# 666DZY666/micronet

Hardware: NVIDIA H100
Metric: qat_step_images_per_sec (higher is better)
Workload: dtype f32 (bf16 tensor-core products of exact integer levels / exact bf16 pieces, fp32 accumulate)

## Files before the change

harness/step_profile.py:

```python
import argparse
import json
import os
import re
import subprocess
import sys

sys.path.insert(0, os.path.dirname(os.path.dirname(os.path.abspath(__file__))))

import torch

from harness import train as H

HEADLINE = "nin_gc_wbwtab_w3a2"


def card():
    try:
        return subprocess.run(["nvidia-smi", "--query-gpu=name,power.limit,clocks.max.sm", "--format=csv,noheader"],
                              capture_output=True, text=True, timeout=30).stdout.strip().splitlines()[0]
    except (OSError, subprocess.SubprocessError, IndexError) as e:
        return f"unknown ({type(e).__name__})"


def producer_bytes(rec, terms_dy):
    n, xb, pooled, plane_only, pk_conv = rec["n"], rec["xb"], rec["pool2"], rec["plane_only"], rec["pk_conv"]
    bits = n / 8
    out = {"channel_stats_kernel": n * xb}
    if pooled:
        out["bn_sign_pool_fwd_kernel"] = n * xb + n + n / 4 + bits
        out["bn_sign_pool_bwd_reduce_kernel"] = n * xb + n + n / 4 + bits
        if pk_conv:
            out["bn_sign_pool_bwd_pack_kernel"] = n * xb + n + n / 4 + bits + 2 * n * terms_dy
        else:
            out["bn_sign_pool_bwd_apply_kernel"] = n * xb + n + n / 4 + bits + 4 * n
    else:
        out["bn_sign_packed_fwd_kernel"] = n * xb + 2 * n + bits + (0 if plane_only else 4 * n)
        out["bn_sign_bwd_reduce_kernel"] = n * xb + 4 * n + bits
        if pk_conv:
            out["bn_sign_bwd_pack_kernel"] = n * xb + 4 * n + bits + 2 * n * terms_dy
        else:
            out["bn_sign_bwd_apply_kernel"] = n * xb + 4 * n + bits + 4 * n
    return out


def base_name(kernel):
    head = kernel.split("(")[0]
    head = re.sub(r"<.*$", "", head)
    return head.split("::")[-1].split(" ")[-1]


def main():
    ap = argparse.ArgumentParser()
    ap.add_argument("--out", required=True)
    ap.add_argument("--steps", type=int, default=5)
    ap.add_argument("--warmup", type=int, default=5)
    ap.add_argument("--batch", type=int, default=256)
    args = ap.parse_args()
    if not torch.cuda.is_available():
        raise SystemExit("step_profile: no CUDA device")
    os.makedirs(args.out, exist_ok=True)
    from micronet_b200 import _lib as L
    from micronet_b200.fused import BatchNormBinarize2d
    w = H.WORKLOADS[HEADLINE]
    dev = torch.device("cuda:0")
    model = H.prepare_engine(H.build_float_model(w["model"]), w["scheme"], **w["prepare"], **w.get("engine_extra", {})).to(dev)
    stepper = H.QatStepper(model, lr=0.01, wd=w["wd"], flat=True, graph=False)
    batches = [H.synthetic_batch(args.batch, w["hw"], seed=100 + i, device=dev) for i in range(2)]
    for i in range(args.warmup):
        stepper.step(*batches[i % 2])
    torch.cuda.synchronize()

    calls = []

    def hook(mod, inp):
        x = inp[0]
        calls.append({"n": x.numel(), "xb": 2 if getattr(x, "_mnb_codes", None) is not None else 4,
                      "pool2": bool(mod.pool2), "plane_only": bool(mod.plane_only) and not mod.pool2,
                      "pk_conv": getattr(x, "_mnb_pk_conv", None) is not None})

    handles = [m.register_forward_pre_hook(hook) for m in model.modules() if isinstance(m, BatchNormBinarize2d)]
    acts = [torch.profiler.ProfilerActivity.CPU, torch.profiler.ProfilerActivity.CUDA]
    with torch.profiler.profile(activities=acts) as prof:
        for i in range(args.steps):
            stepper.step(*batches[i % 2])
        torch.cuda.synchronize()
    for h in handles:
        h.remove()

    terms_dy = min(L.PK_TERMS, L.PK_TERMS_BWD)
    want = {}
    for rec in calls:
        for k, b in producer_bytes(rec, terms_dy).items():
            want[k] = want.get(k, 0.0) + b
    kern = {}
    for e in prof.events():
        if e.device_type != torch.autograd.DeviceType.CUDA:
            continue
        d = kern.setdefault(e.name, {"launches": 0, "us": 0.0})
        d["launches"] += 1
        d["us"] += e.device_time
    rows, total_us = [], sum(d["us"] for d in kern.values()) / args.steps
    for name, d in kern.items():
        row = {"kernel": name, "base": base_name(name), "launches_per_step": d["launches"] / args.steps,
               "us_per_step": d["us"] / args.steps}
        rows.append(row)
    by_base = {}
    for r in rows:
        by_base.setdefault(r["base"], []).append(r)
    for base, rs in by_base.items():
        if base not in want:
            continue
        launches = sum(r["launches_per_step"] for r in rs)
        bytes_step = want[base] / args.steps
        us = sum(r["us_per_step"] for r in rs)
        for r in rs:
            r["bytes_per_launch"] = bytes_step / launches
        rs[0]["group_bytes_per_step"] = bytes_step
        rs[0]["group_GBps"] = bytes_step / (us * 1e-6) / 1e9
    rows.sort(key=lambda r: -r["us_per_step"])
    res = {"card": card(), "workload": HEADLINE, "batch": args.batch, "steps": args.steps,
           "device_us_per_step": total_us, "kernels": rows}
    with open(os.path.join(args.out, "step_profile.json"), "w") as f:
        json.dump(res, f, indent=1)
    lines = [f"card: {res['card']}", f"{HEADLINE}, batch {args.batch}, eager step, {args.steps} profiled steps; "
             f"device time per step {total_us / 1e3:.3f} ms (sum of kernel times)", "",
             f"{'us/step':>9} {'share':>6} {'launch':>6} {'MB/launch':>9} {'GB/s':>7}  kernel"]
    for r in rows:
        mb = f"{r['bytes_per_launch'] / 1e6:9.1f}" if "bytes_per_launch" in r else " " * 9
        gbs = f"{r['group_GBps']:7.0f}" if "group_GBps" in r else " " * 7
        lines.append(f"{r['us_per_step']:9.1f} {r['us_per_step'] / total_us:6.1%} {r['launches_per_step']:6.1f} {mb} {gbs}  "
                     f"{r['kernel'][:110]}")
    txt = "\n".join(lines)
    with open(os.path.join(args.out, "step_profile.txt"), "w") as f:
        f.write(txt + "\n")
    print(txt)


if __name__ == "__main__":
    main()
```

include/micronet_b200.h:

```cpp
#ifndef MICRONET_B200_H
#define MICRONET_B200_H

#include <stdint.h>

#ifdef __cplusplus
extern "C" {
#endif

typedef void* mnb_stream_t;

#define MNB_E_ARG (-1)
#define MNB_E_UNSUPPORTED (-2)

int mnb_version(void);
const char* mnb_last_error(void);
int64_t mnb_launch_count(void);

typedef struct {
  int32_t batch, in_c, in_h, in_w;
  int32_t out_c, ker_h, ker_w;
  int32_t stride_h, stride_w, pad_h, pad_w, dil_h, dil_w, groups;
} mnb_conv_shape;

#define MNB_ACT_DOREFA 1
// ... 103 lines not shown
                    mnb_stream_t stream);
int mnb_bn_sign_bwd(const float* g, const uint32_t* pass_bits, const float* x, int32_t batch, int32_t channels, int32_t hw,
                    const float* mean, const float* invstd, const float* gamma, int32_t training,
                    int32_t out_shuffle_groups, float* dx, float* dgamma, float* dbeta, float* dx_channel_sum,
                    void* scratch, mnb_stream_t stream);

int mnb_bn_sign_pool_fwd(const float* x, int32_t batch, int32_t channels, int32_t H, int32_t W, const float* mean,
                         const float* invstd, const float* gamma, const float* beta, int32_t out_shuffle_groups, float* y,
                         uint32_t* pass_bits, uint8_t* argmax, mnb_stream_t stream);
int mnb_bn_sign_pool_bwd(const float* g, const uint32_t* pass_bits, const uint8_t* argmax, const float* x, int32_t batch,
                         int32_t channels, int32_t H, int32_t W, const float* mean, const float* invstd, const float* gamma,
                         int32_t training, int32_t out_shuffle_groups, float* dx, float* dgamma, float* dbeta,
                         float* dx_channel_sum, void* scratch, mnb_stream_t stream);

int mnb_maxpool2d_fwd(const float* x, int32_t batch, int32_t channels, int32_t H, int32_t W, int32_t kernel, int32_t stride,
                      int32_t pad, int32_t out_shuffle_groups, float* y, uint8_t* argmax, mnb_stream_t stream);
int mnb_maxpool2d_bwd(const float* g, const uint8_t* argmax, int32_t batch, int32_t channels, int32_t H, int32_t W,
                      int32_t kernel, int32_t stride, int32_t pad, int32_t out_shuffle_groups, float* dx,
                      mnb_stream_t stream);

int mnb_bn_sign_fwd_packed(const float* x, int32_t batch, int32_t channels, int32_t hw, const float* mean,
                           const float* invstd, const float* gamma, const float* beta, int32_t out_shuffle_groups, float* y,
                           uint32_t* pass_bits, void* x_packed, mnb_stream_t stream);

int mnb_fconv2d_plan(const mnb_conv_shape* s, int32_t wgrad, int32_t* out, int32_t n);
int mnb_fconv2d_fwd_tc(const mnb_conv_shape* s, const float* x, const float* w, const float* bias, float* y,
                       int32_t* err_flag, mnb_stream_t stream);
int mnb_fconv2d_wg_plan(const mnb_conv_shape* s, int32_t* out, int32_t n);
int mnb_fconv2d_fwd_wg(const mnb_conv_shape* s, const float* x, const float* w, const float* bias, float* y,
                       int32_t* err_flag, mnb_stream_t stream);
int64_t mnb_fconv2d_wgrad_tc_scratch_bytes(const mnb_conv_shape* s);
int64_t mnb_fconv2d_wgrad_wg_scratch_bytes(const mnb_conv_shape* s);
int mnb_fconv2d_wgrad_wg(const mnb_conv_shape* s, const float* dy, const float* x, float* dw, void* scratch,
                         int32_t* err_flag, mnb_stream_t stream);
int mnb_fconv2d_wgrad_tc(const mnb_conv_shape* s, const float* dy, const float* x, float* dw, void* scratch,
                         int32_t* err_flag, mnb_stream_t stream);

int64_t mnb_pk_act_bytes(int32_t batch, int32_t channels, int32_t h, int32_t w, int32_t terms);
int mnb_pk_pack_act(const float* x, int32_t batch, int32_t channels, int32_t h, int32_t w, const mnb_act_qparams* qp,
                    int32_t terms, const float* ch_scale, int32_t phase_split, void* out_pk, uint8_t* bits8,
                    mnb_stream_t stream);
int mnb_bn_relu_quant_pack_fwd(const float* x, int32_t batch, int32_t channels, int32_t hw, const float* mean,
                               const float* invstd, const float* gamma, const float* beta, const mnb_act_qparams* qp,
                               int32_t out_shuffle_groups, void* x_packed, uint32_t* pass_bits, mnb_stream_t stream);
int mnb_bn_sign_bwd_pack(const float* g, const uint32_t* pass_bits, const float* x, int32_t batch, int32_t channels, int32_t hw,
                         const float* mean, const float* invstd, const float* gamma, const float* dgamma, const float* dbeta,
                         int32_t out_shuffle_groups, const float* ch_scale, int32_t terms, float* dx, void* dy_packed,
                         mnb_stream_t stream);
int mnb_bn_sign_pool_bwd_pack(const float* g, const uint32_t* pass_bits, const uint8_t* argmax, const float* x, int32_t batch,
                              int32_t channels, int32_t H, int32_t W, const float* mean, const float* invstd,
                              const float* gamma, const float* dgamma, const float* dbeta, int32_t out_shuffle_groups,
                              const float* ch_scale, int32_t terms, void* dy_packed, mnb_stream_t stream);
int mnb_pk_conv_codes(const mnb_conv_shape* s, const void* a_pk, int32_t terms_a, const void* w_img, int32_t terms_w,
                      const float* n_scale, const float* a_scale, float a_scale_const, const float* bias, int32_t level_bound,
                      int16_t* codes, float* dec, int32_t* err_flag, mnb_stream_t stream);
int mnb_codes_decode(const int16_t* codes, const float* dec, int32_t batch, int32_t channels, int32_t hw, float* x,
                     mnb_stream_t stream);
int mnb_bn_batch_stats_codes(const int16_t* codes, const float* dec, int32_t batch, int32_t channels, int32_t hw, double eps,
                             double momentum, float* running_mean, float* running_var, int64_t* num_batches_tracked,
                             float* mean_invstd, void* scratch, mnb_stream_t stream);
int mnb_bn_sign_fwd_packed_codes(const int16_t* codes, const float* dec, int32_t batch, int32_t channels, int32_t hw,
                                 const float* mean, const float* invstd, const float* gamma, const float* beta,
                                 int32_t out_shuffle_groups, float* y, uint32_t* pass_bits, void* x_packed, mnb_stream_t stream);
int mnb_bn_sign_bwd_codes(const float* g, const uint32_t* pass_bits, const int16_t* codes, const float* dec, int32_t batch,
                          int32_t channels, int32_t hw, const float* mean, const float* invstd, const float* gamma,
                          int32_t training, int32_t out_shuffle_groups, float* dx, float* dgamma, float* dbeta,
                          float* dx_channel_sum, void* scratch, mnb_stream_t stream);
int mnb_bn_sign_pool_fwd_codes(const int16_t* codes, const float* dec, int32_t batch, int32_t channels, int32_t H, int32_t W,
                               const float* mean, const float* invstd, const float* gamma, const float* beta,
                               int32_t out_shuffle_groups, float* y, uint32_t* pass_bits, uint8_t* argmax, mnb_stream_t stream);
int mnb_bn_sign_pool_bwd_codes(const float* g, const uint32_t* pass_bits, const uint8_t* argmax, const int16_t* codes,
                               const float* dec, int32_t batch, int32_t channels, int32_t H, int32_t W, const float* mean,
                               const float* invstd, const float* gamma, int32_t training, int32_t out_shuffle_groups, float* dx,
                               float* dgamma, float* dbeta, float* dx_channel_sum, void* scratch, mnb_stream_t stream);
int mnb_bn_sign_bwd_pack_codes(const float* g, const uint32_t* pass_bits, const int16_t* codes, const float* dec, int32_t batch,
                               int32_t channels, int32_t hw, const float* mean, const float* invstd, const float* gamma,
                               const float* dgamma, const float* dbeta, int32_t out_shuffle_groups, const float* ch_scale,
                               int32_t terms, float* dx, void* dy_packed, mnb_stream_t stream);
int mnb_bn_sign_pool_bwd_pack_codes(const float* g, const uint32_t* pass_bits, const uint8_t* argmax, const int16_t* codes,
                                    const float* dec, int32_t batch, int32_t channels, int32_t H, int32_t W, const float* mean,
                                    const float* invstd, const float* gamma, const float* dgamma, const float* dbeta,
                                    int32_t out_shuffle_groups, const float* ch_scale, int32_t terms, void* dy_packed,
                                    mnb_stream_t stream);
int mnb_pk_pack_act_relu(const float* x, int32_t batch, int32_t channels, int32_t h, int32_t w, const mnb_act_qparams* qp,
                         int32_t terms, const float* ch_scale, int32_t phase_split, int32_t relu, void* out_pk,
                         uint8_t* bits8, mnb_stream_t stream);
int64_t mnb_pk_grouped_act_bytes(int32_t batch, int32_t channels, int32_t h, int32_t w, int32_t terms, int32_t groups);
int mnb_pk_pack_act_grouped(const float* x, int32_t batch, int32_t channels, int32_t h, int32_t w, const mnb_act_qparams* qp,
                            int32_t terms, const float* ch_scale, int32_t phase_split, int32_t relu, void* out_pk,
                            uint8_t* bits8, int32_t groups, mnb_stream_t stream);
int mnb_pk_conv_plan(const mnb_conv_shape* s, int32_t mode, int32_t terms_a, int32_t terms_w, int32_t* out16);
int mnb_pk_conv_plan_ex(const mnb_conv_shape* s, int32_t mode, int32_t terms_a, int32_t terms_w, int32_t* out, int32_t n);
int mnb_pk_wgrad_plan(const mnb_conv_shape* s, int32_t terms_dy, int32_t terms_x, int32_t* out, int32_t n);
int64_t mnb_pk_wimage_bytes(const mnb_conv_shape* s, int32_t mode, int32_t terms_a, int32_t terms_w);
int mnb_pk_pack_weight(const mnb_conv_shape* s, int32_t mode, int32_t terms_a, int32_t terms_w, const int16_t* w_int,
                       const float* w_f32, const float* kzero, void* w_img, mnb_stream_t stream);
int mnb_pk_conv(const mnb_conv_shape* s, int32_t mode, const void* a_pk, int32_t terms_a, const void* w_img, int32_t terms_w,
                const float* n_scale, const float* a_scale, float a_scale_const, const float* bias, const uint8_t* bits8,
                float gain, float* out, int32_t* err_flag, mnb_stream_t stream);
typedef struct mnb_pk_post {
  const mnb_act_qparams* q;
  int32_t relu;
  int32_t phase_split;
  void* out_pk;
  const float* bn_mean;
  const float* bn_invstd;
  const float* bn_gamma;
  const float* bn_beta;
  int32_t shuffle_groups;
  int32_t terms_out;
} mnb_pk_post;
int mnb_pk_conv_post(const mnb_conv_shape* s, const void* a_pk, int32_t terms_a, const void* w_img, int32_t terms_w,
                     const float* n_scale, const float* a_scale, float a_scale_const, const float* bias, float* out,
                     const mnb_pk_post* post, int32_t* err_flag, mnb_stream_t stream);
int mnb_quant_add_pack_fwd(const float* a, const float* b, int32_t batch, int32_t channels, int32_t h, int32_t w,
                           const mnb_act_qparams* qp, int32_t relu, float* out, const mnb_pk_post* post, mnb_stream_t stream);
int mnb_pk_conv_post_plan(const mnb_conv_shape* s, int32_t terms_a, int32_t terms_w, int32_t cpu, const mnb_pk_post* post,
                          int32_t* out, int32_t n);
int64_t mnb_pk_i8_act_bytes(int32_t batch, int32_t channels, int32_t h, int32_t w);
int mnb_pk_i8_pack_act(const float* x, int32_t batch, int32_t channels, int32_t h, int32_t w, const mnb_act_qparams* qp,
                       int32_t phase_split, int32_t relu, void* out_pk, mnb_stream_t stream);
int mnb_pk_i8_conv_plan(const mnb_conv_shape* s, int32_t* out, int32_t n);
int64_t mnb_pk_i8_wimage_bytes(const mnb_conv_shape* s);
int mnb_pk_i8_pack_weight(const mnb_conv_shape* s, const int16_t* w_int, void* w_img, mnb_stream_t stream);
int mnb_pk_i8_conv(const mnb_conv_shape* s, const void* a_pk, const void* w_img, const float* n_scale, const float* a_scale,
                   float a_scale_const, const float* bias, float* out, const mnb_pk_post* post, int32_t* err_flag,
                   mnb_stream_t stream);
int mnb_quant_add_pack_i8_fwd(const float* a, const float* b, int32_t batch, int32_t channels, int32_t h, int32_t w,
                              const mnb_act_qparams* qp, int32_t relu, float* out, const mnb_pk_post* post, mnb_stream_t stream);
int mnb_bn_relu_quant_pack_i8_fwd(const float* x, int32_t batch, int32_t channels, int32_t hw, const float* mean,
                                  const float* invstd, const float* gamma, const float* beta, const mnb_act_qparams* qp,
                                  int32_t out_shuffle_groups, void* x_packed, mnb_stream_t stream);
int mnb_pk_plane_maxpool(const void* in_pk, int32_t batch, int32_t channels, int32_t h, int32_t w, int32_t k, int32_t s, int32_t p,
                         int32_t int8, void* out_pk, mnb_stream_t stream);
int mnb_pk_plane_maxpool_requant(const void* in_pk, int32_t batch, int32_t channels, int32_t h, int32_t w, int32_t k, int32_t s,
                                 int32_t p, int32_t int8, const mnb_act_qparams* q_in, const mnb_act_qparams* q_out, void* out_pk,
                                 mnb_stream_t stream);
int mnb_pk_plane_maxpool_terms(const void* in_pk, int32_t batch, int32_t channels, int32_t h, int32_t w, int32_t k, int32_t s,
                               int32_t p, int32_t terms, void* out_pk, mnb_stream_t stream);
int mnb_bn_relu_pack_terms_fwd(const float* x, int32_t batch, int32_t channels, int32_t hw, const float* mean,
                               const float* invstd, const float* gamma, const float* beta, int32_t relu,
                               int32_t out_shuffle_groups, int32_t terms, void* x_packed, mnb_stream_t stream);
int64_t mnb_pk_wgrad_scratch_bytes(const mnb_conv_shape* s, int32_t terms_dy, int32_t terms_x);
int mnb_pk_wgrad(const mnb_conv_shape* s, const void* dy_pk, int32_t terms_dy, const void* x_pk, int32_t terms_x,
                 const float* a_scale, const float* kdiv, float* dw, void* scratch, int32_t* err_flag, mnb_stream_t stream);
int mnb_pk_wgrad_taps_plan(const mnb_conv_shape* s, int32_t terms_dy, int32_t terms_x, int32_t* out, int32_t n);
int mnb_pk_wgrad_taps(const mnb_conv_shape* s, const void* dy_pk, int32_t terms_dy, const void* x_pk, int32_t terms_x,
                      const float* a_scale, const float* kdiv, float* dw, void* scratch, int32_t* err_flag, mnb_stream_t stream);
int mnb_pk_gc3_plan(const mnb_conv_shape* s, int32_t mode, int32_t terms_a, int32_t terms_w, int32_t* out, int32_t n);
int mnb_pk_gc3_conv(const mnb_conv_shape* s, int32_t mode, const void* a_pk, int32_t terms_a, const void* w_img, int32_t terms_w,
                    const float* n_scale, const float* a_scale, float a_scale_const, const float* bias, const uint8_t* bits8,
                    float gain, float* out, int32_t* err_flag, mnb_stream_t stream);
int mnb_pk_gc3_conv_codes(const mnb_conv_shape* s, const void* a_pk, int32_t terms_a, const void* w_img, int32_t terms_w,
                          const float* n_scale, const float* a_scale, float a_scale_const, const float* bias, int32_t level_bound,
                          int16_t* codes, float* dec, int32_t* err_flag, mnb_stream_t stream);

int mnb_xnor_supported(const mnb_conv_shape* s);
int64_t mnb_xnor_act_bytes(int32_t batch, int32_t channels, int32_t h, int32_t w, int32_t groups);
int mnb_xnor_pack_act(const float* x, int32_t batch, int32_t channels, int32_t h, int32_t w, int32_t groups, void* out_bits,
                      mnb_stream_t stream);
int64_t mnb_xnor_wimage_bytes(const mnb_conv_shape* s);
int mnb_xnor_pack_weight(const mnb_conv_shape* s, const int16_t* w_int, void* w_img, mnb_stream_t stream);
int mnb_xnor_conv_fwd(const mnb_conv_shape* s, const void* a_bits, const void* w_img, const float* alpha, const float* bias,
                      float* y, mnb_stream_t stream);
#define MNB_XNOR_BITS 0
#define MNB_XNOR_PM1_BF16 1
// ... 53 lines not shown
```

micronet_b200/_lib.py:

```python
from __future__ import annotations

import ctypes as C
import os

import torch

_HERE = os.path.dirname(os.path.abspath(__file__))
LIB_PATH = os.path.join(_HERE, "lib", "libmicronet_b200.so")

ACT_DOREFA, ACT_IAO, ACT_SIGN = 1, 2, 3


class ConvShape(C.Structure):
    _fields_ = [(n, C.c_int32) for n in (
        "batch", "in_c", "in_h", "in_w", "out_c", "ker_h", "ker_w", "stride_h", "stride_w",
        "pad_h", "pad_w", "dil_h", "dil_w", "groups")]


class ActQParams(C.Structure):
    _fields_ = [("mode", C.c_int32), ("bits", C.c_int32), ("qmin", C.c_int32), ("qmax", C.c_int32),
                ("q_type", C.c_int32), ("scale", C.c_void_p), ("zero_point", C.c_void_p),
                ("obs_min", C.c_void_p), ("obs_max", C.c_void_p)]


# ... 14 lines not shown
class ConvOperands(C.Structure):
    _fields_ = [("a_codes", C.c_void_p), ("a_f32", C.c_void_p), ("a_offset", C.c_int32),
                ("a_offset_zp", C.c_void_p), ("a_scale", C.c_void_p), ("w_int", C.c_void_p),
                ("w_scale", C.c_void_p), ("w_f32", C.c_void_p), ("bias", C.c_void_p)]


_P, _I, _L, _D = C.c_void_p, C.c_int32, C.c_int64, C.c_double
_SHAPE, _ACTQ, _OPS = C.POINTER(ConvShape), C.POINTER(ActQParams), C.POINTER(ConvOperands)

PROTOTYPES = {
    "mnb_version": (C.c_int, []),
    "mnb_last_error": (C.c_char_p, []),
    "mnb_launch_count": (_L, []),
    "mnb_act_quant_fwd": (C.c_int, [_P, _L, _ACTQ, _P, _P, _P, _P]),
    "mnb_act_quant_bwd": (C.c_int, [_P, _P, _L, _ACTQ, _P, _P]),
    "mnb_bn_fold_fwd": (C.c_int, [_P, _I, _I, _P, _P, _P, _P, _P, _D, _P, _P, _P]),
    "mnb_bn_fold_bwd": (C.c_int, [_P, _P, _P, _I, _I, _P, _P, _P, _P, _D, _P, _P, _P]),
    "mnb_bn_fold_running": (C.c_int, [_P, _P, _P, _P, _I, _D, _I, _P]),
    "mnb_quant_add_fwd": (C.c_int, [_P, _P, _L, _ACTQ, _P, _P, _P, _I, _P]),
    "mnb_quant_add_bwd": (C.c_int, [_P, _P, _P, _L, _ACTQ, _P, _P, _P]),
    "mnb_observe_scratch_bytes": (_L, [_L, _I]),
    "mnb_iao_observe": (C.c_int, [_P, _L, _I, _I, _I, _D, _D, _P, _P, _I, _I, _I, _I, _P, _P, _P, _P]),
    "mnb_iao_update_qparams": (C.c_int, [_P, _P, _I, _I, _I, _I, _P, _P, _P]),
    "mnb_dorefa_weight_fwd": (C.c_int, [_P, _L, _I, _I, _P, _P, _P, _P, _P, _P]),
    "mnb_dorefa_weight_bwd": (C.c_int, [_P, _P, _L, _I, _P, _P, _P]),
    "mnb_wb_weight_fwd": (C.c_int, [_P, _I, _I, _I, _I, _P, _P, _P, _P, _P]),
    "mnb_wb_weight_bwd": (C.c_int, [_P, _P, _P, _I, _I, _I, _I, _P, _P]),
    "mnb_iao_weight_fwd": (C.c_int, [_P, _L, _I, _I, _P, _P, _P, _P, _I, _I, _I, _P, _P, _P, _P, _P]),
    "mnb_iao_weight_bwd": (C.c_int, [_P, _P, _P, _L, _I, _I, _P, _P]),
    "mnb_conv2d_fwd": (C.c_int, [_SHAPE, _OPS, _P, _P]),
    "mnb_conv2d_dgrad": (C.c_int, [_SHAPE, _P, _P, _P, _ACTQ, _P, _P]),
    "mnb_wgrad_scratch_bytes": (_L, [_SHAPE]),
    "mnb_conv2d_wgrad": (C.c_int, [_SHAPE, _P, _OPS, _P, _P, _P]),
    "mnb_channel_stats": (C.c_int, [_P, _I, _I, _I, _I, _P, _P, _P]),
    "mnb_channel_stats_bwd": (C.c_int, [_P, _P, _P, _P, _I, _I, _I, _P, _P]),
    "mnb_fq_conv2d_fwd_tc": (C.c_int, [_SHAPE, _P, _ACTQ, _P, _P, _P, _P, _P, _P, _P, _P, _P]),
    "mnb_conv2d_dgrad_tc": (C.c_int, [_SHAPE, _P, _P, _P, _P, _ACTQ, _P, _P, _P, _P]),
    "mnb_tc_conv_plan": (C.c_int, [_SHAPE, _I, _I, _P, _I]),
    "mnb_wgrad_tc_scratch_bytes": (_L, [_SHAPE]),
    "mnb_wgrad_tc_plan": (C.c_int, [_SHAPE, _I, _P, _I]),
    "mnb_conv2d_wgrad_tc": (C.c_int, [_SHAPE, _P, _P, _ACTQ, _P, _P, _P, _P, _P]),
    "mnb_conv2d_wgrad_cond": (C.c_int, [_SHAPE, _P, _OPS, _P, _P, _P, _P]),
    "mnb_bn_batch_stats": (C.c_int, [_P, _I, _I, _I, _D, _D, _P, _P, _P, _P, _P, _P]),
    "mnb_bn_sign_fwd": (C.c_int, [_P, _I, _I, _I, _P, _P, _P, _P, _I, _P, _P, _P]),
    "mnb_bn_sign_bwd": (C.c_int, [_P, _P, _P, _I, _I, _I, _P, _P, _P, _I, _I, _P, _P, _P, _P, _P, _P]),
    "mnb_bn_sign_pool_fwd": (C.c_int, [_P, _I, _I, _I, _I, _P, _P, _P, _P, _I, _P, _P, _P, _P]),
    "mnb_bn_sign_pool_bwd": (C.c_int, [_P, _P, _P, _P, _I, _I, _I, _I, _P, _P, _P, _I, _I, _P, _P, _P, _P, _P, _P]),
    "mnb_bn_sign_fwd_packed": (C.c_int, [_P, _I, _I, _I, _P, _P, _P, _P, _I, _P, _P, _P, _P]),
    "mnb_fconv2d_plan": (C.c_int, [_SHAPE, _I, _P, _I]),
    "mnb_fconv2d_fwd_tc": (C.c_int, [_SHAPE, _P, _P, _P, _P, _P, _P]),
    "mnb_fconv2d_wg_plan": (C.c_int, [_SHAPE, _P, _I]),
    "mnb_fconv2d_fwd_wg": (C.c_int, [_SHAPE, _P, _P, _P, _P, _P, _P]),
    "mnb_fconv2d_wgrad_tc_scratch_bytes": (_L, [_SHAPE]),
    "mnb_fconv2d_wgrad_tc": (C.c_int, [_SHAPE, _P, _P, _P, _P, _P, _P]),
    "mnb_fconv2d_wgrad_wg_scratch_bytes": (_L, [_SHAPE]),
    "mnb_fconv2d_wgrad_wg": (C.c_int, [_SHAPE, _P, _P, _P, _P, _P, _P]),
    "mnb_maxpool2d_fwd": (C.c_int, [_P, _I, _I, _I, _I, _I, _I, _I, _I, _P, _P, _P]),
    "mnb_maxpool2d_bwd": (C.c_int, [_P, _P, _I, _I, _I, _I, _I, _I, _I, _I, _P, _P]),
    "mnb_adam_step": (C.c_int, [_P, _P, _P, _P, _L, C.c_float, C.c_float, C.c_float, C.c_float, C.c_float, _I, _P]),
    "mnb_pk_act_bytes": (_L, [_I, _I, _I, _I, _I]),
    "mnb_pk_pack_act": (C.c_int, [_P, _I, _I, _I, _I, _ACTQ, _I, _P, _I, _P, _P, _P]),
    "mnb_bn_relu_quant_pack_fwd": (C.c_int, [_P, _I, _I, _I, _P, _P, _P, _P, _ACTQ, _I, _P, _P, _P]),
    "mnb_pk_pack_act_relu": (C.c_int, [_P, _I, _I, _I, _I, _ACTQ, _I, _P, _I, _I, _P, _P, _P]),
    "mnb_pk_grouped_act_bytes": (_L, [_I, _I, _I, _I, _I, _I]),
    "mnb_pk_pack_act_grouped": (C.c_int, [_P, _I, _I, _I, _I, _ACTQ, _I, _P, _I, _I, _P, _P, _I, _P]),
    "mnb_pk_conv_plan": (C.c_int, [_SHAPE, _I, _I, _I, _P]),
    "mnb_pk_conv_plan_ex": (C.c_int, [_SHAPE, _I, _I, _I, _P, _I]),
    "mnb_pk_wgrad_plan": (C.c_int, [_SHAPE, _I, _I, _P, _I]),
    "mnb_pk_wimage_bytes": (_L, [_SHAPE, _I, _I, _I]),
    "mnb_pk_pack_weight": (C.c_int, [_SHAPE, _I, _I, _I, _P, _P, _P, _P, _P]),
    "mnb_pk_conv": (C.c_int, [_SHAPE, _I, _P, _I, _P, _I, _P, _P, C.c_float, _P, _P, C.c_float, _P, _P, _P]),
    "mnb_bn_sign_bwd_pack": (C.c_int, [_P, _P, _P, _I, _I, _I, _P, _P, _P, _P, _P, _I, _P, _I, _P, _P, _P]),
    "mnb_bn_sign_pool_bwd_pack": (C.c_int, [_P, _P, _P, _P, _I, _I, _I, _I, _P, _P, _P, _P, _P, _I, _P, _I, _P, _P]),
    "mnb_pk_conv_post": (C.c_int, [_SHAPE, _P, _I, _P, _I, _P, _P, C.c_float, _P, _P, C.POINTER(PkPost), _P, _P]),
    "mnb_pk_conv_post_plan": (C.c_int, [_SHAPE, _I, _I, _I, C.POINTER(PkPost), _P, _I]),
    "mnb_pk_conv_codes": (C.c_int, [_SHAPE, _P, _I, _P, _I, _P, _P, C.c_float, _P, _I, _P, _P, _P, _P]),
    "mnb_codes_decode": (C.c_int, [_P, _P, _I, _I, _I, _P, _P]),
    "mnb_bn_batch_stats_codes": (C.c_int, [_P, _P, _I, _I, _I, _D, _D, _P, _P, _P, _P, _P, _P]),
    "mnb_bn_sign_fwd_packed_codes": (C.c_int, [_P, _P, _I, _I, _I, _P, _P, _P, _P, _I, _P, _P, _P, _P]),
    "mnb_bn_sign_bwd_codes": (C.c_int, [_P, _P, _P, _P, _I, _I, _I, _P, _P, _P, _I, _I, _P, _P, _P, _P, _P, _P]),
    "mnb_bn_sign_pool_fwd_codes": (C.c_int, [_P, _P, _I, _I, _I, _I, _P, _P, _P, _P, _I, _P, _P, _P, _P]),
    "mnb_bn_sign_pool_bwd_codes": (C.c_int, [_P, _P, _P, _P, _P, _I, _I, _I, _I, _P, _P, _P, _I, _I, _P, _P, _P, _P, _P, _P]),
    "mnb_bn_sign_bwd_pack_codes": (C.c_int, [_P, _P, _P, _P, _I, _I, _I, _P, _P, _P, _P, _P, _I, _P, _I, _P, _P, _P]),
    "mnb_bn_sign_pool_bwd_pack_codes": (C.c_int, [_P, _P, _P, _P, _P, _I, _I, _I, _I, _P, _P, _P, _P, _P, _I, _P, _I, _P,
                                                  _P]),
    "mnb_quant_add_pack_fwd": (C.c_int, [_P, _P, _I, _I, _I, _I, _ACTQ, _I, _P, C.POINTER(PkPost), _P]),
    "mnb_pk_i8_act_bytes": (_L, [_I, _I, _I, _I]),
    "mnb_pk_i8_pack_act": (C.c_int, [_P, _I, _I, _I, _I, _ACTQ, _I, _I, _P, _P]),
    "mnb_pk_i8_conv_plan": (C.c_int, [_SHAPE, _P, _I]),
    "mnb_pk_i8_wimage_bytes": (_L, [_SHAPE]),
    "mnb_pk_i8_pack_weight": (C.c_int, [_SHAPE, _P, _P, _P]),
    "mnb_pk_i8_conv": (C.c_int, [_SHAPE, _P, _P, _P, _P, C.c_float, _P, _P, C.POINTER(PkPost), _P, _P]),
    "mnb_quant_add_pack_i8_fwd": (C.c_int, [_P, _P, _I, _I, _I, _I, _ACTQ, _I, _P, C.POINTER(PkPost), _P]),
    "mnb_bn_relu_quant_pack_i8_fwd": (C.c_int, [_P, _I, _I, _I, _P, _P, _P, _P, _ACTQ, _I, _P, _P]),
    "mnb_pk_plane_maxpool": (C.c_int, [_P, _I, _I, _I, _I, _I, _I, _I, _I, _P, _P]),
    "mnb_pk_plane_maxpool_requant": (C.c_int, [_P, _I, _I, _I, _I, _I, _I, _I, _I, _ACTQ, _ACTQ, _P, _P]),
    "mnb_pk_plane_maxpool_terms": (C.c_int, [_P, _I, _I, _I, _I, _I, _I, _I, _I, _P, _P]),
    "mnb_bn_relu_pack_terms_fwd": (C.c_int, [_P, _I, _I, _I, _P, _P, _P, _P, _I, _I, _I, _P, _P]),
    "mnb_pk_wgrad_scratch_bytes": (_L, [_SHAPE, _I, _I]),
    "mnb_pk_wgrad": (C.c_int, [_SHAPE, _P, _I, _P, _I, _P, _P, _P, _P, _P, _P]),
    "mnb_pk_wgrad_taps_plan": (C.c_int, [_SHAPE, _I, _I, _P, _I]),
    "mnb_pk_wgrad_taps": (C.c_int, [_SHAPE, _P, _I, _P, _I, _P, _P, _P, _P, _P, _P]),
    "mnb_pk_gc3_plan": (C.c_int, [_SHAPE, _I, _I, _I, _P, _I]),
    "mnb_pk_gc3_conv": (C.c_int, [_SHAPE, _I, _P, _I, _P, _I, _P, _P, C.c_float, _P, _P, C.c_float, _P, _P, _P]),
    "mnb_pk_gc3_conv_codes": (C.c_int, [_SHAPE, _P, _I, _P, _I, _P, _P, C.c_float, _P, _I, _P, _P, _P, _P]),
    "mnb_xnor_supported": (C.c_int, [_SHAPE]),
    "mnb_xnor_act_bytes": (_L, [_I, _I, _I, _I, _I]),
    "mnb_xnor_pack_act": (C.c_int, [_P, _I, _I, _I, _I, _I, _P, _P]),
    "mnb_xnor_wimage_bytes": (_L, [_SHAPE]),
    "mnb_xnor_pack_weight": (C.c_int, [_SHAPE, _P, _P, _P]),
    "mnb_xnor_conv_fwd": (C.c_int, [_SHAPE, _P, _P, _P, _P, _P, _P]),
    "mnb_xnor_post_bytes": (_L, [_SHAPE, C.POINTER(XnorPost)]),
    "mnb_xnor_conv_post": (C.c_int, [_SHAPE, _P, _P, _P, _P, C.POINTER(XnorPost), _P, _P]),
    "mnb_xnor_pack_act_post": (C.c_int, [_P, _I, _I, _I, _I, C.POINTER(XnorPost), _P, _P]),
    "mnb_xnor_plan": (C.c_int, [_SHAPE, C.POINTER(XnorPost), _P]),
    "mnb_b1_supported": (C.c_int, [_SHAPE]),
    "mnb_b1_act_bytes": (_L, [_I, _I, _I, _I, _I]),
    "mnb_b1_pack_act": (C.c_int, [_P, _I, _I, _I, _I, _I, _P, _P]),
    "mnb_b1_pack_act_post": (C.c_int, [_P, _I, _I, _I, _I, C.POINTER(XnorPost), _P, _P]),
    "mnb_b1_wimage_bytes": (_L, [_SHAPE]),
    "mnb_b1_pack_weight": (C.c_int, [_SHAPE, _P, _P, _P]),
    "mnb_b1_conv_fwd": (C.c_int, [_SHAPE, _P, _P, _P, _P, _P, _P, _P]),
    "mnb_b1_plan": (C.c_int, [_SHAPE, C.POINTER(XnorPost), _P]),
    "mnb_b1_post_bytes": (_L, [_SHAPE, C.POINTER(XnorPost)]),
    "mnb_b1_conv_post": (C.c_int, [_SHAPE, _P, _P, _P, _P, C.POINTER(XnorPost), _P, _P, _P]),
    "mnb_b1_plane_maxpool": (C.c_int, [_P, _I, _I, _I, _I, _I, _I, _I, _I, _P, _P]),
    "mnb_set_tc_profile_buffer": (None, [_P]),
    "mnb_selftest_mma_rate": (C.c_int, [_I, _I, _I, _I, _I, _P, _P, _P]),
    "mnb_selftest_umma": (C.c_int, [_P, _P, _P, _I, _I, _I, _P, _P]),
    "mnb_selftest_tma3d": (C.c_int, [_P, C.POINTER(C.c_int64), C.POINTER(C.c_int32), C.POINTER(C.c_int32), _P, _P, _P]),
}

_lib = None


def load():
    global _lib
    if _lib is not None:
        return _lib
    if not os.path.exists(LIB_PATH):
        raise RuntimeError(
            f"micronet_b200: {LIB_PATH} is missing - build it with `python -m micronet_b200.build` "
            "(there is no CPU / PyTorch fallback for the fake-quant hot path)")
    lib = C.CDLL(LIB_PATH)
    for name, (res, args) in PROTOTYPES.items():
        fn = getattr(lib, name)
        fn.restype, fn.argtypes = res, args
    _lib = lib
    return lib


def check(rc: int, what: str):
    if rc != 0:
        msg = load().mnb_last_error().decode(errors="replace")
        kind = ValueError if rc < 0 else RuntimeError
        raise kind(f"micronet_b200.{what} failed (code {rc}): {msg}")


def ptr(t):
    return None if t is None else t.data_ptr()


def stream():
    return torch.cuda.current_stream().cuda_stream


def require_cuda(*tensors):
    for t in tensors:
        if t is not None and not t.is_cuda:
            raise RuntimeError(
                "micronet_b200: the fake-quant engine runs on CUDA (sm_90a) tensors only; "
                "got a CPU tensor - there is deliberately no CPU fallback")


def require_f32(*tensors):
    for t in tensors:
        if t is not None and t.dtype != torch.float32:
            raise TypeError(f"micronet_b200: fp32 tensors only (the reference's QAT modules are fp32), got {t.dtype}")


def launch_count() -> int:
    return int(load().mnb_launch_count())


_errflags = {}


def tc_err_flag(device):
    key = (device.type, device.index)
    if key not in _errflags:
        _errflags[key] = torch.zeros(1, dtype=torch.int32, device=device)
    return _errflags[key]


def tc_check(device=None):
    for key, flag in _errflags.items():
        code = int(flag.item())
        if code:
            raise RuntimeError(f"micronet_b200: tensor-core pipeline wait timed out (code {code}) on {key}")


E_UNSUPPORTED = -2
KEEP_DEBUG = False
USE_TC = os.environ.get("MNB_DISABLE_TC", "0") != "1"
PK_MODE = os.environ.get("MNB_PK", "auto")
PK_TERMS = int(os.environ.get("MNB_PK_TERMS", "3"))
PK_TERMS_BWD = int(os.environ.get("MNB_PK_TERMS_BWD", "2"))
PK_WBWTAB = os.environ.get("MNB_PK_WBWTAB", "1") == "1"
PK_WG_TAPS = os.environ.get("MNB_PK_WG_TAPS", "1") != "0"
PK_GC3 = os.environ.get("MNB_PK_GC3", "1") != "0"

XNOR_MODE = os.environ.get("MNB_XNOR", "auto")

PLANE_ONLY = os.environ.get("MNB_PLANE_ONLY", "1") == "1"

_scratch = {}


def scratch(device, rows=1):
    lib = load()
    need = int(lib.mnb_observe_scratch_bytes(0, int(rows)))
    key = (device.type, device.index)
    buf = _scratch.get(key)
    if buf is None or buf.numel() < need:
        buf = torch.zeros(max(need, 1 << 20), dtype=torch.uint8, device=device)
        _scratch[key] = buf
    return buf
```

micronet_b200/csrc/mnb_common.cuh:

```cuda
#pragma once
#include <cuda_runtime.h>
#include <float.h>
#include <stdint.h>

#include "../../include/micronet_b200.h"

int mnb_fail(int code, const char* fmt, ...);
void mnb_count_launches(int n);

#define MNB_REQUIRE(cond, ...)                            \
  do {                                                    \
    if (!(cond)) return mnb_fail(MNB_E_ARG, __VA_ARGS__); \
  } while (0)

#define MNB_LAUNCHED(nlaunch)                                                        \
  do {                                                                               \
    mnb_count_launches(nlaunch);                                                     \
    cudaError_t e__ = cudaGetLastError();                                            \
    if (e__ != cudaSuccess) return mnb_fail((int)e__, "%s:%d launch failed: %s", __FILE__, __LINE__, \
                                            cudaGetErrorString(e__));                \
  } while (0)

static inline int mnb_ceil_div(int64_t a, int64_t b) { return (int)((a + b - 1) / b); }
constexpr int MNB_NUM_SMS = 132;


__device__ __forceinline__ float mnb_round_half_away(float v) {
  float r = floorf(__fadd_rn(fabsf(v), 0.5f));
  return v > 0.f ? r : (v < 0.f ? -r : 0.f);
}
__device__ __forceinline__ float mnb_sign0(float v) { return v > 0.f ? 1.f : (v < 0.f ? -1.f : 0.f); }

__device__ __forceinline__ uint32_t mnb_f2ord(float f) {
  uint32_t u = __float_as_uint(f);
  return (u & 0x80000000u) ? ~u : (u | 0x80000000u);
}
__device__ __forceinline__ float mnb_ord2f(uint32_t u) {
  return __uint_as_float((u & 0x80000000u) ? (u & 0x7fffffffu) : ~u);
}

template <typename T, typename Op>
__device__ __forceinline__ T mnb_warp_reduce(T v, Op op) {
#pragma unroll
  for (int o = 16; o > 0; o >>= 1) v = op(v, __shfl_xor_sync(0xffffffffu, v, o));
  return v;
}
template <typename T, typename Op>
__device__ __forceinline__ T mnb_block_reduce(T v, Op op, T identity, T* smem) {
  const int lane = threadIdx.x & 31, wid = threadIdx.x >> 5;
  v = mnb_warp_reduce(v, op);
  __syncthreads();
  if (lane == 0) smem[wid] = v;
  __syncthreads();
  const int nw = (blockDim.x + 31) >> 5;
  T r = (lane < nw) ? smem[lane] : identity;
  r = mnb_warp_reduce(r, op);
  return r;
}
struct MnbMin { template <typename T> __device__ T operator()(T a, T b) const { return a < b ? a : b; } };
struct MnbMax { template <typename T> __device__ T operator()(T a, T b) const { return a > b ? a : b; } };
struct MnbSum { template <typename T> __device__ T operator()(T a, T b) const { return a + b; } };

__device__ __forceinline__ float bn_bwd_centre(float g, float db, float xhat, float dg) {
  return fmaf(-xhat, dg, __fsub_rn(g, db));
}

struct XDec { float s, b; };
template <typename XT> struct XVec;
template <> struct XVec<float> { typedef float t1; typedef float2 t2; typedef float4 t4; };
template <> struct XVec<int16_t> { typedef short t1; typedef short2 t2; typedef short4 t4; };

template <typename XT>
__device__ __forceinline__ XDec x_dec(const float* dec, int channels, int c) {
  if constexpr (sizeof(XT) == 4) return XDec{1.f, 0.f};
  else return XDec{__ldg(dec + c), __ldg(dec + channels + c)};
}
template <typename XT>
__device__ __forceinline__ float x_val(XT q, XDec d) {
  if constexpr (sizeof(XT) == 4) return q;
  else return fmaf((float)q, d.s, d.b);
}
template <int VEC, typename XT>
__device__ __forceinline__ void x_load(const XT* p, XDec d, float (&v)[VEC]) {
  if constexpr (VEC == 1) {
    v[0] = x_val<XT>(__ldg(reinterpret_cast<const typename XVec<XT>::t1*>(p)), d);
  } else if constexpr (VEC == 2) {
    const typename XVec<XT>::t2 t = __ldg(reinterpret_cast<const typename XVec<XT>::t2*>(p));
    v[0] = x_val<XT>(t.x, d); v[1] = x_val<XT>(t.y, d);
  } else {
    static_assert(VEC == 4, "x_load: 1, 2 or 4 elements");
    const typename XVec<XT>::t4 t = __ldg(reinterpret_cast<const typename XVec<XT>::t4*>(p));
    v[0] = x_val<XT>(t.x, d); v[1] = x_val<XT>(t.y, d); v[2] = x_val<XT>(t.z, d); v[3] = x_val<XT>(t.w, d);
  }
}
template <typename XT>
__device__ __forceinline__ float4 x_load4(const XT* p, XDec d) {
  float v[4];
  x_load<4>(p, d, v);
  return make_float4(v[0], v[1], v[2], v[3]);
}

struct MnbActQ {
  int mode, qmin, qmax;
  float s, zp, lo, hi;
  float rinv;
};

// ... 171 lines not shown
```

micronet_b200/csrc/mnb_fused.cu:

```cuda
#include <algorithm>

#include "mnb_common.cuh"

static inline cudaStream_t S(mnb_stream_t s) { return (cudaStream_t)s; }
constexpr int FUSED_SPLITS = 32;

__device__ __forceinline__ uint32_t shuffled_channel(uint32_t c, uint32_t sg, uint32_t cpg) {
  return sg > 1 ? (c % cpg) * sg + c / cpg : c;
}

__global__ void __launch_bounds__(256) bn_sign_fwd_v4_kernel(const float4* __restrict__ x, uint32_t n4, uint32_t channels,
                                                             uint32_t hw4, uint32_t sg, const float* __restrict__ mean,
                                                             const float* __restrict__ invstd, const float* __restrict__ gamma,
                                                             const float* __restrict__ beta, float4* __restrict__ y,
                                                             uint32_t* __restrict__ bits) {
  const uint32_t lane = threadIdx.x & 31;
  const uint32_t stride = gridDim.x * blockDim.x;
  const uint32_t n4_up = (n4 + 31u) & ~31u;
  const uint32_t cpg = channels / sg;
  for (uint32_t i = blockIdx.x * blockDim.x + threadIdx.x; i < n4_up; i += stride) {
    uint32_t nib = 0;
    if (i < n4) {
      const uint32_t plane = i / hw4, off = i - plane * hw4;
      const uint32_t b = plane / channels, c = plane - b * channels;
      const float mu = __ldg(mean + c), sc = __ldg(gamma + c) * __ldg(invstd + c), be = __ldg(beta + c);
      const float4 v = __ldg(x + i);
      const float b0 = fmaf(v.x - mu, sc, be), b1 = fmaf(v.y - mu, sc, be), b2 = fmaf(v.z - mu, sc, be),
                  b3 = fmaf(v.w - mu, sc, be);
      const uint32_t o = (b * channels + shuffled_channel(c, sg, cpg)) * hw4 + off;
      y[o] = make_float4(b0 < 0.f ? -1.f : 1.f, b1 < 0.f ? -1.f : 1.f, b2 < 0.f ? -1.f : 1.f, b3 < 0.f ? -1.f : 1.f);
      nib = (uint32_t)(fabsf(b0) < 1.f) | ((uint32_t)(fabsf(b1) < 1.f) << 1) | ((uint32_t)(fabsf(b2) < 1.f) << 2) |
            ((uint32_t)(fabsf(b3) < 1.f) << 3);
    }
    uint32_t w = nib << (4 * (lane & 7));
    w |= __shfl_xor_sync(0xffffffffu, w, 1);
    w |= __shfl_xor_sync(0xffffffffu, w, 2);
    w |= __shfl_xor_sync(0xffffffffu, w, 4);
    if ((lane & 7) == 0 && i < n4) bits[i >> 3] = w;
  }
}

__global__ void __launch_bounds__(256) bn_sign_fwd_kernel(const float* __restrict__ x, int64_t n, int channels, int hw,
                                                          int sg, const float* __restrict__ mean,
                                                          const float* __restrict__ invstd, const float* __restrict__ gamma,
                                                          const float* __restrict__ beta, float* __restrict__ y,
                                                          uint32_t* __restrict__ bits) {
  const int lane = threadIdx.x & 31;
  const int64_t warp = ((int64_t)blockIdx.x * blockDim.x + threadIdx.x) >> 5;
  const int64_t nwarps = ((int64_t)gridDim.x * blockDim.x) >> 5;
  const uint32_t cpg = (uint32_t)(channels / sg);
  for (int64_t base = warp * 32; base < n; base += nwarps * 32) {
    const int64_t i = base + lane;
    bool pass = false;
    if (i < n) {
      const int64_t plane = i / hw;
      const int c = (int)(plane % channels);
      const float sc = __ldg(gamma + c) * __ldg(invstd + c);
      const float bn = fmaf(__ldg(x + i) - __ldg(mean + c), sc, __ldg(beta + c));
      pass = fabsf(bn) < 1.f;
      const int64_t o = (plane - c + shuffled_channel((uint32_t)c, (uint32_t)sg, cpg)) * hw + (i - plane * hw);
      y[o] = bn < 0.f ? -1.f : 1.f;
    }
    const uint32_t word = __ballot_sync(0xffffffffu, pass);
    if (lane == 0) bits[base >> 5] = word;
  }
}

template <bool VEC, typename XT>
__global__ void __launch_bounds__(256) bn_sign_bwd_reduce_kernel(const float* __restrict__ g, const uint32_t* __restrict__ bits,
                                                                 const XT* __restrict__ x, const float* __restrict__ dec,
                                                                 int batch, int channels, int hw,
                                                                 int sg, const float* __restrict__ mean,
                                                                 const float* __restrict__ invstd, float* __restrict__ dgamma,
                                                                 float* __restrict__ dbeta, uint32_t* counters,
                                                                 double* partial) {
  __shared__ double red[32];
  __shared__ bool last;
  const int c = blockIdx.x, sp = blockIdx.y, nsp = gridDim.y;
  const int oc = (int)shuffled_channel((uint32_t)c, (uint32_t)sg, (uint32_t)(channels / sg));
  const float mu = __ldg(mean + c), is = __ldg(invstd + c);
  const XDec d = x_dec<XT>(dec, channels, c);
  const int b_lo = (int)((int64_t)batch * sp / nsp), b_hi = (int)((int64_t)batch * (sp + 1) / nsp);
  double s1, s2;
  if (VEC) {
    const uint32_t hw4 = (uint32_t)hw >> 2, total = (uint32_t)(b_hi - b_lo) * hw4;
    const float4* g4 = reinterpret_cast<const float4*>(g);
    float f1[2] = {0.f, 0.f}, f2[2] = {0.f, 0.f};
    for (uint32_t t0 = threadIdx.x; t0 < total; t0 += 2 * blockDim.x) {
#pragma unroll
      for (int u = 0; u < 2; ++u) {
        const uint32_t t = t0 + u * blockDim.x;
        if (t < total) {
          const uint32_t b = t / hw4, i = t - b * hw4;
          const uint32_t fi4 = ((uint32_t)(b_lo + b) * channels + c) * hw4 + i;
          const uint32_t go4 = ((uint32_t)(b_lo + b) * channels + oc) * hw4 + i;
          const uint32_t nib = (__ldg(bits + (fi4 >> 3)) >> (4 * (fi4 & 7))) & 15u;
          const float4 gv = __ldg(g4 + go4), xv = x_load4(x + 4 * fi4, d);
          const float g0 = (nib & 1u) ? gv.x : 0.f, g1 = (nib & 2u) ? gv.y : 0.f, g2 = (nib & 4u) ? gv.z : 0.f,
                      g3 = (nib & 8u) ? gv.w : 0.f;
          f1[u] += (g0 + g1) + (g2 + g3);
          f2[u] += (g0 * ((xv.x - mu) * is) + g1 * ((xv.y - mu) * is)) + (g2 * ((xv.z - mu) * is) + g3 * ((xv.w - mu) * is));
        }
      }
    }
    s1 = (double)f1[0] + (double)f1[1];
    s2 = (double)f2[0] + (double)f2[1];
  } else {
    s1 = 0.0; s2 = 0.0;
    for (int b = b_lo; b < b_hi; ++b) {
      const int64_t off = ((int64_t)b * channels + c) * hw, goff = ((int64_t)b * channels + oc) * hw;
      float f1 = 0.f, f2 = 0.f;
      for (int i = threadIdx.x; i < hw; i += blockDim.x) {
        const int64_t fi = off + i;
        const bool pass = (__ldg(bits + (fi >> 5)) >> (fi & 31)) & 1u;
        const float gv = pass ? __ldg(g + goff + i) : 0.f;
        f1 += gv;
        f2 += gv * ((x_val<XT>(__ldg(x + fi), d) - mu) * is);
      }
      s1 += (double)f1; s2 += (double)f2;
    }
  }
  s1 = mnb_block_reduce(s1, MnbSum(), 0.0, red);
  s2 = mnb_block_reduce(s2, MnbSum(), 0.0, red);
  if (threadIdx.x == 0) {
    partial[((int64_t)c * nsp + sp) * 2 + 0] = s1;
    partial[((int64_t)c * nsp + sp) * 2 + 1] = s2;
    __threadfence();
    last = (atomicAdd(counters + c, 1u) == (uint32_t)nsp - 1);
  }
  __syncthreads();
  if (!last || threadIdx.x != 0) return;
  __threadfence();
  s1 = 0.0; s2 = 0.0;
  for (int j = 0; j < nsp; ++j) { s1 += partial[((int64_t)c * nsp + j) * 2]; s2 += partial[((int64_t)c * nsp + j) * 2 + 1]; }
  dbeta[c] = (float)s1;
  dgamma[c] = (float)s2;
  counters[c] = 0;
}

template <bool VEC, typename XT>
__global__ void __launch_bounds__(256) bn_sign_bwd_apply_kernel(const float* __restrict__ g, const uint32_t* __restrict__ bits,
                                                                const XT* __restrict__ x, const float* __restrict__ dec,
                                                                int batch, int channels, int hw,
                                                                int sg, float inv_count, const float* __restrict__ mean,
                                                                const float* __restrict__ invstd, const float* __restrict__ gamma,
                                                                const float* __restrict__ dgamma, const float* __restrict__ dbeta,
                                                                int training, float* __restrict__ dx, float* __restrict__ dx_sum,
                                                                uint32_t* counters, double* partial) {
  __shared__ double red[32];
  __shared__ bool last;
  const int c = blockIdx.x, sp = blockIdx.y, nsp = gridDim.y;
  const int oc = (int)shuffled_channel((uint32_t)c, (uint32_t)sg, (uint32_t)(channels / sg));
  const float mu = __ldg(mean + c), is = __ldg(invstd + c), k = __ldg(gamma + c) * is;
  const float db = training ? __ldg(dbeta + c) * inv_count : 0.f, dg = training ? __ldg(dgamma + c) * inv_count : 0.f;
  const XDec d = x_dec<XT>(dec, channels, c);
  const int b_lo = (int)((int64_t)batch * sp / nsp), b_hi = (int)((int64_t)batch * (sp + 1) / nsp);
  double s;
  if (VEC) {
    const uint32_t hw4 = (uint32_t)hw >> 2, total = (uint32_t)(b_hi - b_lo) * hw4;
    const float4* g4 = reinterpret_cast<const float4*>(g);
    float4* dx4 = reinterpret_cast<float4*>(dx);
    float f[2] = {0.f, 0.f};
    for (uint32_t t0 = threadIdx.x; t0 < total; t0 += 2 * blockDim.x) {
#pragma unroll
      for (int u = 0; u < 2; ++u) {
        const uint32_t t = t0 + u * blockDim.x;
        if (t < total) {
          const uint32_t b = t / hw4, i = t - b * hw4;
          const uint32_t fi4 = ((uint32_t)(b_lo + b) * channels + c) * hw4 + i;
          const uint32_t go4 = ((uint32_t)(b_lo + b) * channels + oc) * hw4 + i;
          const uint32_t nib = (__ldg(bits + (fi4 >> 3)) >> (4 * (fi4 & 7))) & 15u;
          const float4 gv = __ldg(g4 + go4);
          float v0 = (nib & 1u) ? gv.x : 0.f, v1 = (nib & 2u) ? gv.y : 0.f, v2 = (nib & 4u) ? gv.z : 0.f,
                v3 = (nib & 8u) ? gv.w : 0.f;
          if (training) {
            const float4 xv = x_load4(x + 4 * fi4, d);
            v0 = bn_bwd_centre(v0, db, (xv.x - mu) * is, dg);
            v1 = bn_bwd_centre(v1, db, (xv.y - mu) * is, dg);
            v2 = bn_bwd_centre(v2, db, (xv.z - mu) * is, dg);
            v3 = bn_bwd_centre(v3, db, (xv.w - mu) * is, dg);
          }
          const float4 o = make_float4(k * v0, k * v1, k * v2, k * v3);
          dx4[fi4] = o;
          f[u] += (o.x + o.y) + (o.z + o.w);
        }
      }
    }
    s = (double)f[0] + (double)f[1];
  } else {
    s = 0.0;
    for (int b = b_lo; b < b_hi; ++b) {
      const int64_t off = ((int64_t)b * channels + c) * hw, goff = ((int64_t)b * channels + oc) * hw;
      float f = 0.f;
      for (int i = threadIdx.x; i < hw; i += blockDim.x) {
        const int64_t fi = off + i;
        const bool pass = (__ldg(bits + (fi >> 5)) >> (fi & 31)) & 1u;
        float v = pass ? __ldg(g + goff + i) : 0.f;
        if (training) v = bn_bwd_centre(v, db, (x_val<XT>(__ldg(x + fi), d) - mu) * is, dg);
        v = k * v;
        dx[fi] = v;
        f += v;
      }
      s += (double)f;
    }
  }
  if (!dx_sum) return;
  s = mnb_block_reduce(s, MnbSum(), 0.0, red);
  if (threadIdx.x == 0) {
    partial[((int64_t)c * nsp + sp) * 2] = s;
    __threadfence();
    last = (atomicAdd(counters + c, 1u) == (uint32_t)nsp - 1);
  }
  __syncthreads();
  if (!last || threadIdx.x != 0) return;
  __threadfence();
  s = 0.0;
  for (int j = 0; j < nsp; ++j) s += partial[((int64_t)c * nsp + j) * 2];
  dx_sum[c] = (float)s;
  counters[c] = 0;
}

template <typename XT = float>
static bool planes_vectorizable(int64_t n, int hw, const void* a, const void* b, const void* c, const XT* x = nullptr) {
  return (hw & 3) == 0 && n < (1ll << 31) &&
         (((uintptr_t)a | (uintptr_t)b | (uintptr_t)c) & 15) == 0 && ((uintptr_t)x & (4 * sizeof(XT) - 1)) == 0;
}
static int plane_splits(int batch, int64_t per, int channels) {
  const int64_t want = (2 * 8 * MNB_NUM_SMS + channels - 1) / channels;
  return (int)std::max<int64_t>(1, std::min<int64_t>(std::min<int64_t>(std::min<int64_t>(FUSED_SPLITS, batch), per / 2048), want));
}

extern "C" int mnb_bn_sign_fwd(const float* x, int32_t batch, int32_t channels, int32_t hw, const float* mean,
                               const float* invstd, const float* gamma, const float* beta, int32_t out_shuffle_groups,
                               float* y, uint32_t* pass_bits, mnb_stream_t stream) {
  MNB_REQUIRE(x && mean && invstd && gamma && beta && y && pass_bits, "NULL bn_sign_fwd pointer");
  MNB_REQUIRE(batch > 0 && channels > 0 && hw > 0, "bad bn_sign_fwd shape");
  MNB_REQUIRE(out_shuffle_groups >= 1 && channels % out_shuffle_groups == 0, "shuffle groups %d do not divide %d channels",
              out_shuffle_groups, channels);
  const int64_t n = (int64_t)batch * channels * hw;
  int blocks = (int)std::min<int64_t>(mnb_ceil_div(n, 256 * 4), MNB_NUM_SMS * 8);
  if (planes_vectorizable(n, hw, x, y, nullptr))
    bn_sign_fwd_v4_kernel<<<blocks, 256, 0, S(stream)>>>(reinterpret_cast<const float4*>(x), (uint32_t)(n / 4),
                                                         (uint32_t)channels, (uint32_t)(hw / 4), (uint32_t)out_shuffle_groups,
                                                         mean, invstd, gamma, beta, reinterpret_cast<float4*>(y), pass_bits);
  else
    bn_sign_fwd_kernel<<<blocks, 256, 0, S(stream)>>>(x, n, channels, hw, out_shuffle_groups, mean, invstd, gamma, beta, y,
                                                      pass_bits);
  MNB_LAUNCHED(1);
  return 0;
}

template <typename XT>
static int bn_sign_bwd(const float* g, const uint32_t* pass_bits, const XT* x, const float* dec, int32_t batch, int32_t channels,
                       int32_t hw, const float* mean, const float* invstd, const float* gamma, int32_t training,
                       int32_t out_shuffle_groups, float* dx, float* dgamma, float* dbeta, float* dx_channel_sum, void* scratch,
                       mnb_stream_t stream) {
  MNB_REQUIRE(g && pass_bits && x && mean && invstd && gamma && dx && dgamma && dbeta && scratch, "NULL bn_sign_bwd pointer");
  MNB_REQUIRE(batch > 0 && channels > 0 && channels <= 8192 && hw > 0, "bad bn_sign_bwd shape");
  MNB_REQUIRE(out_shuffle_groups >= 1 && channels % out_shuffle_groups == 0, "shuffle groups %d do not divide %d channels",
              out_shuffle_groups, channels);
  const int64_t n = (int64_t)batch * channels * hw;
  const int64_t per = (int64_t)batch * hw;
  const int splits = plane_splits(batch, per, channels);
  uint32_t* counters = reinterpret_cast<uint32_t*>(reinterpret_cast<char*>(scratch) + 16384);
  double* partial = reinterpret_cast<double*>(reinterpret_cast<char*>(scratch) + 49152);
  const dim3 grid(channels, splits);
  const float inv_count = 1.f / (float)per;
  if (planes_vectorizable(n, hw, g, dx, nullptr, x)) {
    bn_sign_bwd_reduce_kernel<true, XT><<<grid, 256, 0, S(stream)>>>(g, pass_bits, x, dec, batch, channels, hw, out_shuffle_groups,
                                                                     mean, invstd, dgamma, dbeta, counters, partial);
    if (training == 2) { MNB_LAUNCHED(1); return 0; }
    bn_sign_bwd_apply_kernel<true, XT><<<grid, 256, 0, S(stream)>>>(g, pass_bits, x, dec, batch, channels, hw, out_shuffle_groups,
                                                                    inv_count, mean, invstd, gamma, dgamma, dbeta, training, dx,
                                                                    dx_channel_sum, counters, partial);
  } else {
    bn_sign_bwd_reduce_kernel<false, XT><<<grid, 256, 0, S(stream)>>>(g, pass_bits, x, dec, batch, channels, hw, out_shuffle_groups,
                                                                      mean, invstd, dgamma, dbeta, counters, partial);
    if (training == 2) { MNB_LAUNCHED(1); return 0; }
    bn_sign_bwd_apply_kernel<false, XT><<<grid, 256, 0, S(stream)>>>(g, pass_bits, x, dec, batch, channels, hw, out_shuffle_groups,
                                                                     inv_count, mean, invstd, gamma, dgamma, dbeta, training, dx,
                                                                     dx_channel_sum, counters, partial);
  }
  MNB_LAUNCHED(2);
  return 0;
}

extern "C" int mnb_bn_sign_bwd(const float* g, const uint32_t* pass_bits, const float* x, int32_t batch, int32_t channels,
                               int32_t hw, const float* mean, const float* invstd, const float* gamma, int32_t training,
                               int32_t out_shuffle_groups, float* dx, float* dgamma, float* dbeta, float* dx_channel_sum,
                               void* scratch, mnb_stream_t stream) {
  return bn_sign_bwd<float>(g, pass_bits, x, nullptr, batch, channels, hw, mean, invstd, gamma, training, out_shuffle_groups, dx,
                            dgamma, dbeta, dx_channel_sum, scratch, stream);
}

extern "C" int mnb_bn_sign_bwd_codes(const float* g, const uint32_t* pass_bits, const int16_t* codes, const float* dec,
                                     int32_t batch, int32_t channels, int32_t hw, const float* mean, const float* invstd,
                                     const float* gamma, int32_t training, int32_t out_shuffle_groups, float* dx, float* dgamma,
                                     float* dbeta, float* dx_channel_sum, void* scratch, mnb_stream_t stream) {
  MNB_REQUIRE(dec, "NULL decode pair");
  return bn_sign_bwd<int16_t>(g, pass_bits, codes, dec, batch, channels, hw, mean, invstd, gamma, training, out_shuffle_groups, dx,
                              dgamma, dbeta, dx_channel_sum, scratch, stream);
}

struct PoolGeom { uint32_t channels, H, W4, OH, OW2, sg; };

__device__ __forceinline__ uint32_t first_max_of_signs(bool p0, bool p1, bool p2, bool p3) {
  return p0 ? 0u : (p1 ? 1u : (p2 ? 2u : (p3 ? 3u : 0u)));
}

template <typename XT>
__global__ void __launch_bounds__(256) bn_sign_pool_fwd_kernel(const XT* __restrict__ x, const float* __restrict__ dec,
                                                               uint32_t n_pairs, PoolGeom gm,
                                                               const float* __restrict__ mean, const float* __restrict__ invstd,
                                                               const float* __restrict__ gamma, const float* __restrict__ beta,
// ... 422 lines not shown
```

micronet_b200/csrc/mnb_pk.cu:

```cuda
#include <cuda.h>
#include <cuda_bf16.h>

#include <algorithm>
#include <cstdlib>
#include <cstring>

#include "mnb_common.cuh"
#include "mnb_tc.cuh"

namespace pk {

constexpr int MAXST = 8;
constexpr int MAXTAP = 64, MAXTMPL = 16, MAXY = 4, MAXPAIR = 6, MAXPROG = 512;
constexpr int kSmemBudget = 227 * 1024 - 3072;
constexpr int kNtSizes[] = {16, 32, 48, 64, 96, 128};

struct Tmpl { int kph, tap0, ntap, blk_off, blk_bytes; };

struct Plan {
  int mode;
  int B, G, R, S, stride;
  int HA, WA, C8A, nkph;
  int kg, ng, NOUT;
  int OHr, OWr, OH, OW, omul, ny;
  int hlo, hhi, wlo, whi;
  int Wt, BW, TH, THH, TB, npos, col_tiles, row_tiles, img_tiles, n_mtiles;
  int Nt, n_ntiles, MT, n_mgroups, n_items;
  int CC, ksteps, chunks;
  int TA, TBk, npairs, pair_a[MAXPAIR], pair_b[MAXPAIR];
  int ntmpl[MAXY], ntap[MAXY];
  Tmpl tmpl[MAXY][MAXTMPL];
  int tap_aoff[MAXY][MAXTAP];
  short tap_r[MAXY][MAXTAP], tap_s[MAXY][MAXTAP];
  int img_bytes[MAXY], y_off[MAXY];
  int64_t wimg_bytes;
  int a_box_bytes, a_bytes, b_off, stage_bytes, nstage, st_log2, smem_bytes, off_stg;
  int segmented, seg_len;
  int cpu;
};

static inline int ceil_div(int a, int b) { return (a + b - 1) / b; }
static inline int round_up(int a, int b) { return ceil_div(a, b) * b; }

static void make_pairs(int TA, int TBk, Plan& p) {
  const int lim = std::max(TA, TBk) - 1;
  p.npairs = 0;
  for (int sum = lim; sum >= 0; --sum)
    for (int a = 0; a < TA; ++a) {
      const int b = sum - a;
      if (b < 0 || b >= TBk) continue;
      if (p.npairs < MAXPAIR) { p.pair_a[p.npairs] = a; p.pair_b[p.npairs] = b; ++p.npairs; }
    }
}

static int unsupported(const char* why) { return mnb_fail(MNB_E_UNSUPPORTED, "pk conv: %s", why); }

static int make_plan(const mnb_conv_shape* s, int mode, int TA, int TBk, Plan& p, int cpu = 8) {
  MNB_REQUIRE(s != nullptr, "conv shape is NULL");
  memset(&p, 0, sizeof(p));
  const int C = s->in_c, K = s->out_c, G = s->groups, H = s->in_h, W = s->in_w, R = s->ker_h, S = s->ker_w;
  MNB_REQUIRE(s->batch > 0 && C > 0 && K > 0 && H > 0 && W > 0 && G > 0 && C % G == 0 && K % G == 0 && R > 0 && S > 0,
              "bad conv shape");
  MNB_REQUIRE(TA >= 1 && TA <= 3 && TBk >= 1 && TBk <= 3, "term counts must be 1..3");
  MNB_REQUIRE(cpu == 8 || (cpu == 16 && mode == 0 && TA == 1 && TBk == 1), "int8 plans are single-product forward plans");
  if (s->dil_h != 1 || s->dil_w != 1) return unsupported("dilation != 1");
  if (s->stride_h != s->stride_w || (s->stride_h != 1 && s->stride_h != 2)) return unsupported("stride must be 1 or 2");
  const int st = s->stride_h, ph_ = s->pad_h, pw_ = s->pad_w;
  if (ph_ > R - 1 || pw_ > S - 1) return unsupported("padding larger than the filter");
  const int P = (H + 2 * ph_ - R) / st + 1, Q = (W + 2 * pw_ - S) / st + 1;
  if (P < 1 || Q < 1) return unsupported("empty output");
  if (st == 2 && ((H | W) & 1)) return unsupported("stride 2 needs even H and W");
  const int cin_g = C / G, cout_g = K / G;
  p.mode = mode; p.B = s->batch; p.G = G; p.R = R; p.S = S; p.stride = st;
  p.TA = TA; p.TBk = TBk; p.cpu = cpu;
  make_pairs(TA, TBk, p);
  if (mode == 0) {
    p.kg = cin_g; p.ng = cout_g; p.NOUT = K;
    p.nkph = st == 2 ? 4 : 1;
    p.HA = H / st; p.WA = W / st; p.C8A = ceil_div(C, cpu);
    p.OHr = P; p.OWr = Q; p.OH = P; p.OW = Q; p.omul = 1; p.ny = 1;
  } else {
    p.kg = cout_g; p.ng = cin_g; p.NOUT = C;
    p.nkph = 1; p.HA = P; p.WA = Q; p.C8A = ceil_div(K, 8);
    p.OHr = H / st; p.OWr = W / st; p.OH = H; p.OW = W; p.omul = st; p.ny = st == 2 ? 4 : 1;
  }
  if (cpu == 16 && G > 1 && (p.kg % cpu)) return unsupported("grouped int8 conv needs GEMM-K channels per group % 16 == 0");
  if (cpu == 8) p.C8A = G * ceil_div(p.kg, 8);
  if (cpu == 16 && (int64_t)p.kg * R * S * 128 * 127 > (int64_t)INT32_MAX) return unsupported("int8 sums could overflow s32");
  struct Tap { int kph, sh, sw, r, s; };
// ... 502 lines not shown
}

__global__ void __launch_bounds__(256) bn_relu_pack_terms_kernel(const float* __restrict__ x, int batch, int channels, int hw,
                                                                 int sg, const float* __restrict__ mean,
                                                                 const float* __restrict__ invstd,
                                                                 const float* __restrict__ gamma,
                                                                 const float* __restrict__ beta, int relu, int terms,
                                                                 uint4* __restrict__ xp) {
  const int c8n = channels / 8, cpg = channels / sg;
  const int64_t total = (int64_t)batch * c8n * hw;
  for (int64_t idx = (int64_t)blockIdx.x * blockDim.x + threadIdx.x; idx < total; idx += (int64_t)gridDim.x * blockDim.x) {
    const int pos = (int)(idx % hw);
    const int64_t t = idx / hw;
    const int oc8 = (int)(t % c8n), b = (int)(t / c8n);
    float v[8];
#pragma unroll
    for (int j = 0; j < 8; ++j) {
      const int oc = oc8 * 8 + j;
      const int c = sg > 1 ? (oc % sg) * cpg + oc / sg : oc;
      float y = __ldg(x + ((int64_t)b * channels + c) * hw + pos);
      if (mean) y = fmaf(__fsub_rn(y, __ldg(mean + c)), __fmul_rn(__ldg(gamma + c), __ldg(invstd + c)), __ldg(beta + c));
      v[j] = relu ? fmaxf(y, 0.f) : y;
    }
    store_terms8(v, terms, xp + idx, total);
  }
}

template <int CPU>
__global__ void __launch_bounds__(256) quant_add_pack_kernel(const float* __restrict__ a, const float* __restrict__ b, int B, int C,
                                                             int H, int W, int C8, mnb_act_qparams qadd, int relu,
                                                             float* __restrict__ out, mnb_act_qparams qnext, int next_relu,
                                                             int phase_split, uint4* __restrict__ out_pk) {
  const MnbActQ q = mnb_load_actq(qadd), qn = mnb_load_actq(qnext);
  const float zpn = (qnext.mode == MNB_ACT_IAO && qnext.zero_point) ? __ldg(qnext.zero_point) : 0.f;
  const uint32_t HW = (uint32_t)H * (uint32_t)W;
  const uint32_t plane = blockIdx.y * blockDim.y + threadIdx.y;
  if (plane >= (uint32_t)B * (uint32_t)C8) return;
  const uint32_t bi = plane / (uint32_t)C8, c8 = plane - bi * (uint32_t)C8;
  for (uint32_t pos = blockIdx.x * blockDim.x + threadIdx.x; pos < HW; pos += gridDim.x * blockDim.x) {
    const int64_t base = ((int64_t)bi * C + c8 * CPU) * HW + pos;
    float va[CPU], vb[CPU], lev[CPU];
#pragma unroll
    for (int j = 0; j < CPU; ++j) {
      const bool live = (int)c8 * CPU + j < C;
      va[j] = live ? __ldg(a + base + (int64_t)j * HW) : 0.f;
      vb[j] = live ? __ldg(b + base + (int64_t)j * HW) : 0.f;
    }
    float la[CPU], lb[CPU], sum[CPU];
    uint32_t pbits;
    mnb_act_levels<CPU>(q, va, la, pbits);
    mnb_act_levels<CPU>(q, vb, lb, pbits);
#pragma unroll
    for (int j = 0; j < CPU; ++j) {
      const bool live = (int)c8 * CPU + j < C;
      float oa, ob;
      if (q.mode == MNB_ACT_DOREFA) { oa = __fmul_rn(la[j], q.s); ob = __fmul_rn(lb[j], q.s); }
      else { oa = __fmul_rn(__fadd_rn(la[j], q.zp), q.s); ob = __fmul_rn(__fadd_rn(lb[j], q.zp), q.s); }
      float t = __fadd_rn(oa, ob);
      if (relu) t = fmaxf(t, 0.f);
      if (live) out[base + (int64_t)j * HW] = t;
      sum[j] = next_relu ? fmaxf(t, 0.f) : t;
    }
    mnb_act_levels<CPU>(qn, sum, lev, pbits);
#pragma unroll
    for (int j = 0; j < CPU; ++j) lev[j] = ((int)c8 * CPU + j < C) ? lev[j] + zpn : 0.f;
    int64_t dst;
    if (phase_split) {
      const uint32_t h = pos / (uint32_t)W, w = pos - h * (uint32_t)W;
      const uint32_t oct = ((h & 1u) * 2u + (w & 1u)) * (uint32_t)C8 + c8;
      dst = (((int64_t)bi * 4 * C8 + oct) * (H >> 1) + (h >> 1)) * (W >> 1) + (w >> 1);
    } else {
      dst = (int64_t)plane * HW + pos;
    }
    if constexpr (CPU == 16) out_pk[dst] = pack16_s8(lev);
    else out_pk[dst] = make_uint4(pack2(lev[0], lev[1]), pack2(lev[2], lev[3]), pack2(lev[4], lev[5]), pack2(lev[6], lev[7]));
  }
}

template <int VEC> struct PkVec;
template <> struct PkVec<1> { typedef float type; };
template <> struct PkVec<2> { typedef float2 type; };
template <> struct PkVec<4> { typedef float4 type; };

template <int VEC, typename XT>
__global__ void __launch_bounds__(256) bn_sign_bwd_pack_kernel(const float* __restrict__ g, const uint32_t* __restrict__ bits,
                                                               const XT* __restrict__ x, const float* __restrict__ dec,
                                                               int batch, int channels, int hw,
                                                               int sg, float inv_count, const float* __restrict__ mean,
                                                               const float* __restrict__ invstd, const float* __restrict__ gamma,
                                                               const float* __restrict__ dgamma, const float* __restrict__ dbeta,
                                                               const float* __restrict__ ch_scale, int terms,
                                                               float* __restrict__ dx, uint4* __restrict__ out, int64_t plane_vecs) {
  typedef typename PkVec<VEC>::type T;
  const int lane = threadIdx.x & 31;
  const int c8n = channels / 8, cpg = channels / sg, chunks = hw / (32 * VEC);
  const int64_t items = (int64_t)batch * c8n * chunks;
  const int64_t nwarps = ((int64_t)gridDim.x * blockDim.x) >> 5;
  for (int64_t w = ((int64_t)blockIdx.x * blockDim.x + threadIdx.x) >> 5; w < items; w += nwarps) {
    const int ch = (int)(w % chunks);
    const int64_t pl = w / chunks;
    const int c8 = (int)(pl % c8n), b = (int)(pl / c8n);
    const int pos = (ch * 32 + lane) * VEC;
    T gv[8];
    float xf[8][VEC];
    uint32_t bw[8];
#pragma unroll
    for (int j = 0; j < 8; ++j) {
      const int c = c8 * 8 + j;
      const int oc = sg > 1 ? (c % cpg) * sg + c / cpg : c;
      const int64_t fi = ((int64_t)b * channels + c) * hw + pos;
      gv[j] = __ldg(reinterpret_cast<const T*>(g + ((int64_t)b * channels + oc) * hw + pos));
      x_load<VEC>(x + fi, x_dec<XT>(dec, channels, c), xf[j]);
      bw[j] = __ldg(bits + (fi >> 5)) >> (fi & 31);
    }
    float v[VEC][8];
#pragma unroll
    for (int j = 0; j < 8; ++j) {
      const int c = c8 * 8 + j;
      const float mu = __ldg(mean + c), is = __ldg(invstd + c), k = __ldg(gamma + c) * is;
      const float db = __ldg(dbeta + c) * inv_count, dg = __ldg(dgamma + c) * inv_count;
      const float sc = ch_scale ? __ldg(ch_scale + c) : 1.f;
      const float* gf = reinterpret_cast<const float*>(&gv[j]);
      T dv;
      float* df = reinterpret_cast<float*>(&dv);
#pragma unroll
      for (int i = 0; i < VEC; ++i) {
        float t = ((bw[j] >> i) & 1u) ? gf[i] : 0.f;
        t = bn_bwd_centre(t, db, (xf[j][i] - mu) * is, dg);
        t = k * t;
        df[i] = t;
        v[i][j] = ch_scale ? __fmul_rn(t, sc) : t;
      }
      if (dx) *reinterpret_cast<T*>(dx + ((int64_t)b * channels + c) * hw + pos) = dv;
    }
    const int64_t dst = pl * hw + pos;
    for (int tm = 0; tm < terms; ++tm) {
#pragma unroll
      for (int i = 0; i < VEC; ++i) {
        uint32_t pk4[4];
#pragma unroll
        for (int j = 0; j < 4; ++j) {
          pk4[j] = pack2(v[i][2 * j], v[i][2 * j + 1]);
          v[i][2 * j] -= __uint_as_float(pk4[j] << 16);
          v[i][2 * j + 1] -= __uint_as_float(pk4[j] & 0xffff0000u);
        }
        out[(int64_t)tm * plane_vecs + dst + i] = make_uint4(pk4[0], pk4[1], pk4[2], pk4[3]);
      }
    }
  }
}

template <typename XT>
__global__ void __launch_bounds__(256) bn_sign_pool_bwd_pack_kernel(const float2* __restrict__ g, const uchar2* __restrict__ arg,
                                                                    const uint8_t* __restrict__ bits8, const XT* __restrict__ x,
                                                                    const float* __restrict__ dec, int batch, int channels, int H, int W4, int sg, float inv_count,
                                                                    const float* __restrict__ mean, const float* __restrict__ invstd,
                                                                    const float* __restrict__ gamma, const float* __restrict__ dgamma,
                                                                    const float* __restrict__ dbeta, const float* __restrict__ ch_scale,
                                                                    int terms, uint4* __restrict__ out, int64_t plane_vecs) {
  const uint32_t OH = (uint32_t)H / 2u, OW2 = (uint32_t)W4, c8n = (uint32_t)channels / 8u, cpg = (uint32_t)channels / (uint32_t)sg;
  const uint32_t per_plane = OH * OW2;
  const int64_t total = (int64_t)batch * c8n * per_plane;
  for (int64_t it = (int64_t)blockIdx.x * blockDim.x + threadIdx.x; it < total; it += (int64_t)gridDim.x * blockDim.x) {
    const uint32_t rem = (uint32_t)(it % per_plane);
    const int64_t pl = it / per_plane;
    const uint32_t c8 = (uint32_t)(pl % c8n), b = (uint32_t)(pl / c8n);
    const uint32_t oh = rem / OW2, j = rem - oh * OW2;
    float v[8][8];
#pragma unroll
    for (int q = 0; q < 8; ++q) {
      const uint32_t c = c8 * 8u + q;
      const uint32_t oc = sg > 1 ? (c % cpg) * (uint32_t)sg + c / cpg : c;
      const uint32_t plane = b * (uint32_t)channels + c;
      const float2 gv = __ldg(g + ((size_t)(b * (uint32_t)channels + oc) * OH + oh) * OW2 + j);
      const uchar2 a = arg[((size_t)plane * OH + oh) * OW2 + j];
      const uint32_t i0 = (plane * (uint32_t)H + 2u * oh) * (uint32_t)W4 + j, i1 = i0 + (uint32_t)W4;
      const uint32_t n0 = (bits8[i0 >> 1] >> (4u * (i0 & 1u))) & 15u, n1 = (bits8[i1 >> 1] >> (4u * (i1 & 1u))) & 15u;
      const XDec d = x_dec<XT>(dec, channels, (int)c);
      const float4 r0 = x_load4(x + 4 * i0, d), r1 = x_load4(x + 4 * i1, d);
      const float mu = __ldg(mean + c), is = __ldg(invstd + c), k = __ldg(gamma + c) * is;
      const float db = __ldg(dbeta + c) * inv_count, dg = __ldg(dgamma + c) * inv_count;
      const float sc = ch_scale ? __ldg(ch_scale + c) : 1.f;
      const uint32_t e0 = (a.x >> 1) * 4u + (a.x & 1u), e1 = (a.y >> 1) * 4u + 2u + (a.y & 1u);
      const uint32_t nib = n0 | (n1 << 4);
      const float xs[8] = {r0.x, r0.y, r0.z, r0.w, r1.x, r1.y, r1.z, r1.w};
#pragma unroll
      for (int e = 0; e < 8; ++e) {
        float t = 0.f;
        if ((uint32_t)e == e0 && ((nib >> e) & 1u)) t = gv.x;
        if ((uint32_t)e == e1 && ((nib >> e) & 1u)) t = gv.y;
        t = bn_bwd_centre(t, db, (xs[e] - mu) * is, dg);
        t = k * t;
        v[e][q] = ch_scale ? __fmul_rn(t, sc) : t;
      }
    }
    const int64_t dst0 = (pl * H + 2 * oh) * (int64_t)(4 * W4) + 4 * j;
    for (int tm = 0; tm < terms; ++tm) {
#pragma unroll
      for (int e = 0; e < 8; ++e) {
        uint32_t pk4[4];
#pragma unroll
        for (int q = 0; q < 4; ++q) {
          pk4[q] = pack2(v[e][2 * q], v[e][2 * q + 1]);
          v[e][2 * q] -= __uint_as_float(pk4[q] << 16);
          v[e][2 * q + 1] -= __uint_as_float(pk4[q] & 0xffff0000u);
        }
        out[(int64_t)tm * plane_vecs + dst0 + (e >> 2) * (int64_t)(4 * W4) + (e & 3)] = make_uint4(pk4[0], pk4[1], pk4[2], pk4[3]);
      }
    }
  }
}

struct PackWParams {
  Plan pl;
  const int16_t* w_int; const float* w_f32; const float* kzero;
  int cin_g, cout_g;
};

template <int CPU>
__global__ void __launch_bounds__(256) pack_weight_kernel(const __grid_constant__ PackWParams pp, uint4* __restrict__ out) {
  const Plan& p = pp.pl;
  const int64_t total = p.wimg_bytes / 16;
  const int RS = p.R * p.S;
  for (int64_t v = (int64_t)blockIdx.x * blockDim.x + threadIdx.x; v < total; v += (int64_t)gridDim.x * blockDim.x) {
    int64_t byte = v * 16;
    int y = 0;
    for (int yy = 1; yy < p.ny; ++yy) if (byte >= p.y_off[yy]) y = yy;
    byte -= p.y_off[y];
    if (p.img_bytes[y] == 0) continue;
    const int ntg = (int)(byte / p.img_bytes[y]);
// ... 1274 lines not shown
                     p.segmented, p.segmented ? p.seg_len : 0, p.npairs, p.col_tiles, p.n_mgroups,
                     p.ntmpl[0], p.ntmpl[1], p.ntmpl[2], p.ntmpl[3], p.ntap[0], p.ntap[1], p.ntap[2], p.ntap[3], words, last_seg};
  for (int i = 0; i < std::min(n, 31); ++i) out[i] = v[i];
}

extern "C" int64_t mnb_pk_act_bytes(int32_t batch, int32_t channels, int32_t h, int32_t w, int32_t terms) {
  return (int64_t)terms * batch * ((channels + 7) / 8) * h * w * 16;
}

extern "C" int mnb_pk_pack_act(const float* x, int32_t batch, int32_t channels, int32_t h, int32_t w,
                               const mnb_act_qparams* qp, int32_t terms, const float* ch_scale, int32_t phase_split,
                               void* out_pk, uint8_t* bits8, mnb_stream_t stream) {
  return mnb_pk_pack_act_relu(x, batch, channels, h, w, qp, terms, ch_scale, phase_split, 0, out_pk, bits8, stream);
}

extern "C" int mnb_pk_pack_act_relu(const float* x, int32_t batch, int32_t channels, int32_t h, int32_t w,
                                    const mnb_act_qparams* qp, int32_t terms, const float* ch_scale, int32_t phase_split,
                                    int32_t relu, void* out_pk, uint8_t* bits8, mnb_stream_t stream) {
  MNB_REQUIRE(x && out_pk, "NULL pk_pack_act pointer");
  MNB_REQUIRE(batch > 0 && channels > 0 && h > 0 && w > 0 && terms >= 1 && terms <= 3, "bad pk_pack_act arguments");
  MNB_REQUIRE((reinterpret_cast<uintptr_t>(out_pk) & 15) == 0, "packed tensor must be 16-byte aligned");
  if (phase_split) MNB_REQUIRE(((h | w) & 1) == 0, "phase split needs even H and W");
  const int C8 = (channels + 7) / 8;
  const int64_t plane_vecs = (int64_t)batch * C8 * h * w;
  MNB_REQUIRE((int64_t)batch * C8 <= 65535 * 8 && (int64_t)h * w < (1ll << 31), "pk_pack_act: too many (image, octet) planes");
  dim3 blocks, threads;
  if (!unit_grid(batch, C8, h * w, blocks, threads))
    return mnb_fail(MNB_E_UNSUPPORTED, "pk_pack_act: %d (image, octet) planes exceed the grid", batch * C8);
  cudaStream_t st = (cudaStream_t)stream;
  if (qp) {
    MNB_REQUIRE(qp->mode == MNB_ACT_DOREFA || qp->mode == MNB_ACT_IAO || qp->mode == MNB_ACT_SIGN, "unknown activation quantizer");
    if (qp->mode == MNB_ACT_DOREFA) MNB_REQUIRE(qp->bits >= 2 && qp->bits <= 8, "DoReFa a_bits must be in [2,8]");
    const int a_off = qp->mode == MNB_ACT_IAO ? qp->qmin : (qp->mode == MNB_ACT_SIGN ? -1 : 0);
    pk::pack_act_kernel<1><<<blocks, threads, 0, st>>>(x, batch, channels, h, w, C8, terms, nullptr, *qp, a_off, phase_split,
                                                   reinterpret_cast<uint4*>(out_pk), plane_vecs, bits8, relu);
  } else {
    mnb_act_qparams none{};
    pk::pack_act_kernel<0><<<blocks, threads, 0, st>>>(x, batch, channels, h, w, C8, terms, ch_scale, none, 0, phase_split,
                                                   reinterpret_cast<uint4*>(out_pk), plane_vecs, nullptr, relu);
  }
  MNB_LAUNCHED(1);
  return 0;
}

extern "C" int64_t mnb_pk_grouped_act_bytes(int32_t batch, int32_t channels, int32_t h, int32_t w, int32_t terms, int32_t groups) {
  if (groups < 1 || channels % groups) return -1;
  return (int64_t)terms * batch * groups * ((channels / groups + 7) / 8) * h * w * 16;
}

extern "C" int mnb_pk_pack_act_grouped(const float* x, int32_t batch, int32_t channels, int32_t h, int32_t w,
                                       const mnb_act_qparams* qp, int32_t terms, const float* ch_scale, int32_t phase_split,
                                       int32_t relu, void* out_pk, uint8_t* bits8, int32_t groups, mnb_stream_t stream) {
  MNB_REQUIRE(x && out_pk, "NULL pk_pack_act_grouped pointer");
  MNB_REQUIRE(batch > 0 && channels > 0 && h > 0 && w > 0 && terms >= 1 && terms <= 3 && groups >= 1 && channels % groups == 0,
              "bad pk_pack_act_grouped arguments");
  MNB_REQUIRE((reinterpret_cast<uintptr_t>(out_pk) & 15) == 0, "packed tensor must be 16-byte aligned");
  if (phase_split) MNB_REQUIRE(((h | w) & 1) == 0, "phase split needs even H and W");
  const int cg = channels / groups;
  if (groups == 1 || cg % 8 == 0)
    return mnb_pk_pack_act_relu(x, batch, channels, h, w, qp, terms, ch_scale, phase_split, relu, out_pk, bits8, stream);
  const int kg8 = (cg + 7) / 8, C8 = groups * kg8;
  const int64_t plane_vecs = (int64_t)batch * C8 * h * w;
  MNB_REQUIRE((int64_t)batch * C8 <= 65535 * 8 && (int64_t)h * w < (1ll << 31), "pk_pack_act_grouped: too many (image, octet) planes");
  dim3 blocks, threads;
  if (!unit_grid(batch, C8, h * w, blocks, threads))
    return mnb_fail(MNB_E_UNSUPPORTED, "pk_pack_act_grouped: %d (image, octet) planes exceed the grid", batch * C8);
  cudaStream_t st = (cudaStream_t)stream;
  if (qp) {
    MNB_REQUIRE(qp->mode == MNB_ACT_DOREFA || qp->mode == MNB_ACT_IAO || qp->mode == MNB_ACT_SIGN, "unknown activation quantizer");
    if (qp->mode == MNB_ACT_DOREFA) MNB_REQUIRE(qp->bits >= 2 && qp->bits <= 8, "DoReFa a_bits must be in [2,8]");
    pk::pack_act_grouped_kernel<1><<<blocks, threads, 0, st>>>(x, batch, channels, h, w, C8, terms, nullptr, *qp, phase_split,
                                                               reinterpret_cast<uint4*>(out_pk), plane_vecs, bits8, relu, cg, kg8);
  } else {
    mnb_act_qparams none{};
    pk::pack_act_grouped_kernel<0><<<blocks, threads, 0, st>>>(x, batch, channels, h, w, C8, terms, ch_scale, none, phase_split,
                                                               reinterpret_cast<uint4*>(out_pk), plane_vecs, nullptr, relu, cg,
                                                               kg8);
  }
  MNB_LAUNCHED(1);
  return 0;
}

template <typename XT>
static int bn_sign_bwd_pack(const float* g, const uint32_t* pass_bits, const XT* x, const float* dec, int32_t batch,
                            int32_t channels, int32_t hw, const float* mean, const float* invstd, const float* gamma,
                            const float* dgamma, const float* dbeta, int32_t out_shuffle_groups, const float* ch_scale,
                            int32_t terms, float* dx, void* dy_packed, mnb_stream_t stream) {
  MNB_REQUIRE(g && pass_bits && x && mean && invstd && gamma && dgamma && dbeta && dy_packed, "NULL bn_sign_bwd_pack pointer");
  MNB_REQUIRE(batch > 0 && channels > 0 && hw > 0 && terms >= 1 && terms <= 3, "bad bn_sign_bwd_pack arguments");
  MNB_REQUIRE(out_shuffle_groups >= 1 && channels % out_shuffle_groups == 0, "shuffle groups %d do not divide %d channels",
              out_shuffle_groups, channels);
  if (channels % 8 || (reinterpret_cast<uintptr_t>(dy_packed) & 15))
    return mnb_fail(MNB_E_UNSUPPORTED, "packed BatchNorm backward needs channels %% 8 == 0 and a 16-byte aligned output");
  if (hw % 32) return mnb_fail(MNB_E_UNSUPPORTED, "packed BatchNorm backward needs H*W %% 32 == 0");
  const int c8n = channels / 8;
  auto al = [](const void* p, int a) { return p == nullptr || (reinterpret_cast<uintptr_t>(p) & (uintptr_t)(a - 1)) == 0; };
  constexpr int xs = (int)sizeof(XT);
  const int vec = (hw % 128 == 0 && al(g, 16) && al(x, 4 * xs) && al(dx, 16)) ? 4
                  : ((hw % 64 == 0 && al(g, 8) && al(x, 2 * xs) && al(dx, 8)) ? 2 : 1);
  const int64_t warps = (int64_t)batch * c8n * (hw / (32 * vec));
  const int blocks = (int)std::min<int64_t>(mnb_ceil_div(warps, 8), (int64_t)MNB_NUM_SMS * 8);
  const float inv_count = 1.f / (float)((int64_t)batch * hw);
  uint4* outp = reinterpret_cast<uint4*>(dy_packed);
  const int64_t plane_vecs = (int64_t)batch * c8n * hw;
  cudaStream_t st = (cudaStream_t)stream;
#define MNB_BWD_PACK(V)                                                                                                          \
  pk::bn_sign_bwd_pack_kernel<V, XT><<<blocks, 256, 0, st>>>(g, pass_bits, x, dec, batch, channels, hw, out_shuffle_groups,     \
                                                             inv_count, mean, invstd, gamma, dgamma, dbeta, ch_scale, terms, dx, \
                                                             outp, plane_vecs)
  if (vec == 4) MNB_BWD_PACK(4); else if (vec == 2) MNB_BWD_PACK(2); else MNB_BWD_PACK(1);
#undef MNB_BWD_PACK
  MNB_LAUNCHED(1);
  return 0;
}

extern "C" int mnb_bn_sign_bwd_pack(const float* g, const uint32_t* pass_bits, const float* x, int32_t batch, int32_t channels,
                                    int32_t hw, const float* mean, const float* invstd, const float* gamma, const float* dgamma,
                                    const float* dbeta, int32_t out_shuffle_groups, const float* ch_scale, int32_t terms,
                                    float* dx, void* dy_packed, mnb_stream_t stream) {
  return bn_sign_bwd_pack<float>(g, pass_bits, x, nullptr, batch, channels, hw, mean, invstd, gamma, dgamma, dbeta,
                                 out_shuffle_groups, ch_scale, terms, dx, dy_packed, stream);
}

extern "C" int mnb_bn_sign_bwd_pack_codes(const float* g, const uint32_t* pass_bits, const int16_t* codes, const float* dec,
                                          int32_t batch, int32_t channels, int32_t hw, const float* mean, const float* invstd,
                                          const float* gamma, const float* dgamma, const float* dbeta, int32_t out_shuffle_groups,
                                          const float* ch_scale, int32_t terms, float* dx, void* dy_packed, mnb_stream_t stream) {
  MNB_REQUIRE(dec, "NULL decode pair");
  return bn_sign_bwd_pack<int16_t>(g, pass_bits, codes, dec, batch, channels, hw, mean, invstd, gamma, dgamma, dbeta,
                                   out_shuffle_groups, ch_scale, terms, dx, dy_packed, stream);
}

template <typename XT>
static int bn_sign_pool_bwd_pack(const float* g, const uint32_t* pass_bits, const uint8_t* argmax, const XT* x, const float* dec,
                                 int32_t batch, int32_t channels, int32_t H, int32_t W, const float* mean, const float* invstd,
                                 const float* gamma, const float* dgamma, const float* dbeta, int32_t out_shuffle_groups,
                                 const float* ch_scale, int32_t terms, void* dy_packed, mnb_stream_t stream) {
  MNB_REQUIRE(g && pass_bits && argmax && x && mean && invstd && gamma && dgamma && dbeta && dy_packed, "NULL bn_sign_pool_bwd_pack pointer");
  MNB_REQUIRE(batch > 0 && channels > 0 && H > 0 && W > 0 && terms >= 1 && terms <= 3, "bad bn_sign_pool_bwd_pack arguments");
  MNB_REQUIRE(out_shuffle_groups >= 1 && channels % out_shuffle_groups == 0, "shuffle groups %d do not divide %d channels",
              out_shuffle_groups, channels);
  if ((H & 1) || (W & 7) || channels % 8 || (int64_t)batch * channels * H * W >= (1ll << 31) ||
      (reinterpret_cast<uintptr_t>(x) & (4 * sizeof(XT) - 1)) || (reinterpret_cast<uintptr_t>(dy_packed) & 15) ||
      (reinterpret_cast<uintptr_t>(g) & 7))
    return mnb_fail(MNB_E_UNSUPPORTED, "packed pooled BatchNorm backward needs even H, W %% 8 == 0, channels %% 8 == 0, aligned tensors");
  const int c8n = channels / 8;
  const int64_t total = (int64_t)batch * c8n * (H / 2) * (W / 4);
  const int blocks = (int)std::min<int64_t>(mnb_ceil_div(total, 256), (int64_t)MNB_NUM_SMS * 8);
  pk::bn_sign_pool_bwd_pack_kernel<XT><<<blocks, 256, 0, (cudaStream_t)stream>>>(
      reinterpret_cast<const float2*>(g), reinterpret_cast<const uchar2*>(argmax), reinterpret_cast<const uint8_t*>(pass_bits),
      x, dec, batch, channels, H, W / 4, out_shuffle_groups, 1.f / (float)((int64_t)batch * H * W), mean,
      invstd, gamma, dgamma, dbeta, ch_scale, terms, reinterpret_cast<uint4*>(dy_packed), (int64_t)batch * c8n * H * W);
  MNB_LAUNCHED(1);
  return 0;
}

extern "C" int mnb_bn_sign_pool_bwd_pack(const float* g, const uint32_t* pass_bits, const uint8_t* argmax, const float* x,
                                         int32_t batch, int32_t channels, int32_t H, int32_t W, const float* mean,
                                         const float* invstd, const float* gamma, const float* dgamma, const float* dbeta,
                                         int32_t out_shuffle_groups, const float* ch_scale, int32_t terms, void* dy_packed,
                                         mnb_stream_t stream) {
  return bn_sign_pool_bwd_pack<float>(g, pass_bits, argmax, x, nullptr, batch, channels, H, W, mean, invstd, gamma, dgamma, dbeta,
                                      out_shuffle_groups, ch_scale, terms, dy_packed, stream);
}

extern "C" int mnb_bn_sign_pool_bwd_pack_codes(const float* g, const uint32_t* pass_bits, const uint8_t* argmax,
                                               const int16_t* codes, const float* dec, int32_t batch, int32_t channels, int32_t H,
                                               int32_t W, const float* mean, const float* invstd, const float* gamma,
                                               const float* dgamma, const float* dbeta, int32_t out_shuffle_groups,
                                               const float* ch_scale, int32_t terms, void* dy_packed, mnb_stream_t stream) {
  MNB_REQUIRE(dec, "NULL decode pair");
  return bn_sign_pool_bwd_pack<int16_t>(g, pass_bits, argmax, codes, dec, batch, channels, H, W, mean, invstd, gamma, dgamma,
                                        dbeta, out_shuffle_groups, ch_scale, terms, dy_packed, stream);
}

extern "C" int mnb_quant_add_pack_fwd(const float* a, const float* b, int32_t batch, int32_t channels, int32_t h, int32_t w,
                                      const mnb_act_qparams* qp, int32_t relu, float* out, const mnb_pk_post* post,
                                      mnb_stream_t stream) {
  return quant_add_pack<8>(a, b, batch, channels, h, w, qp, relu, out, post, stream);
}

extern "C" int mnb_bn_relu_quant_pack_fwd(const float* x, int32_t batch, int32_t channels, int32_t hw, const float* mean,
                                          const float* invstd, const float* gamma, const float* beta,
                                          const mnb_act_qparams* qp, int32_t out_shuffle_groups, void* x_packed,
                                          uint32_t* pass_bits, mnb_stream_t stream) {
  MNB_REQUIRE(x && mean && invstd && gamma && beta && qp && x_packed && pass_bits, "NULL bn_relu_quant_pack pointer");
  MNB_REQUIRE(batch > 0 && channels > 0 && hw > 0, "bad bn_relu_quant_pack shape");
  MNB_REQUIRE(qp->mode == MNB_ACT_DOREFA && qp->bits >= 2 && qp->bits <= 8, "the fused producer takes a DoReFa quantizer with 2..8 bits");
  MNB_REQUIRE(out_shuffle_groups >= 1 && channels % out_shuffle_groups == 0, "shuffle groups %d do not divide %d channels",
              out_shuffle_groups, channels);
  if (channels % 8 || hw % 32 || (reinterpret_cast<uintptr_t>(x_packed) & 15))
    return mnb_fail(MNB_E_UNSUPPORTED, "fused producer needs channels %% 8 == 0, H*W %% 32 == 0, 16-byte aligned output");
  const int64_t warps = (int64_t)batch * (channels / 8) * (hw / 32);
  const int blocks = (int)std::min<int64_t>(mnb_ceil_div(warps, 8), (int64_t)MNB_NUM_SMS * 16);
  pk::bn_relu_quant_pack_kernel<<<blocks, 256, 0, (cudaStream_t)stream>>>(x, batch, channels, hw, out_shuffle_groups, mean, invstd,
                                                                       gamma, beta, *qp, pass_bits,
                                                                       reinterpret_cast<uint4*>(x_packed));
  MNB_LAUNCHED(1);
  return 0;
}

extern "C" int mnb_bn_relu_quant_pack_i8_fwd(const float* x, int32_t batch, int32_t channels, int32_t hw, const float* mean,
                                             const float* invstd, const float* gamma, const float* beta,
                                             const mnb_act_qparams* qp, int32_t out_shuffle_groups, void* x_packed,
                                             mnb_stream_t stream) {
  MNB_REQUIRE(x && mean && invstd && gamma && beta && qp && x_packed, "NULL bn_relu_quant_pack_i8 pointer");
  MNB_REQUIRE(batch > 0 && channels > 0 && hw > 0, "bad bn_relu_quant_pack_i8 shape");
  MNB_REQUIRE(out_shuffle_groups >= 1 && channels % out_shuffle_groups == 0, "shuffle groups %d do not divide %d channels",
              out_shuffle_groups, channels);
  if (qp->mode != MNB_ACT_DOREFA || !i8_quantizer(qp))
    return mnb_fail(MNB_E_UNSUPPORTED, "bn_relu_quant_pack_i8: the int8 producer takes a DoReFa quantizer with 2..7 bits");
  if (channels % 16 || hw % 32 || (reinterpret_cast<uintptr_t>(x_packed) & 15))
    return mnb_fail(MNB_E_UNSUPPORTED, "int8 producer needs channels %% 16 == 0, H*W %% 32 == 0, 16-byte aligned output");
// ... 611 lines not shown
```

micronet_b200/csrc/mnb_quant.cu:

```cuda
#include <math.h>
#include <stdarg.h>
#include <stdio.h>

#include <atomic>

#include "mnb_common.cuh"

static thread_local char g_mnb_err[512] = "";
static std::atomic<int64_t> g_mnb_launches{0};

int mnb_fail(int code, const char* fmt, ...) {
  va_list ap;
  va_start(ap, fmt);
  vsnprintf(g_mnb_err, sizeof(g_mnb_err), fmt, ap);
  va_end(ap);
  return code;
}
void mnb_count_launches(int n) { g_mnb_launches.fetch_add(n, std::memory_order_relaxed); }

extern "C" int mnb_version(void) { return 100; }
extern "C" const char* mnb_last_error(void) { return g_mnb_err; }
extern "C" int64_t mnb_launch_count(void) { return g_mnb_launches.load(); }

static inline cudaStream_t S(mnb_stream_t s) { return (cudaStream_t)s; }
// ... 486 lines not shown
                                 int16_t* w_int, float* w_scale, float* wq, float* aux, mnb_stream_t stream) {
  MNB_REQUIRE(w && aux && out_c > 0 && in_c_per_group > 0 && ker_hw > 0, "bad wbwtab weight arguments");
  MNB_REQUIRE(W == 2 || W == 3, "wbwtab W must be 2 (binary) or 3 (ternary), got %d", W);
  wb_weight_fwd_kernel<<<out_c, 128, 0, S(stream)>>>(w, in_c_per_group, ker_hw, W, w_int, w_scale, wq, aux, out_c);
  MNB_LAUNCHED(1);
  return 0;
}

extern "C" int mnb_wb_weight_bwd(const float* g_wq, const float* w, const float* aux, int32_t out_c,
                                 int32_t in_c_per_group, int32_t ker_hw, int32_t W, float* dw,
                                 mnb_stream_t stream) {
  MNB_REQUIRE(g_wq && w && aux && dw && out_c > 0, "bad wbwtab weight-bwd arguments");
  MNB_REQUIRE(W == 2 || W == 3, "wbwtab W must be 2 or 3, got %d", W);
  wb_weight_bwd_kernel<<<out_c, 128, 0, S(stream)>>>(g_wq, w, aux, in_c_per_group * ker_hw, W, out_c, dw);
  MNB_LAUNCHED(1);
  return 0;
}

__global__ void __launch_bounds__(256) iao_weight_fwd_kernel(const float* __restrict__ w, int64_t n, int64_t inner,
                                                             int out_c, int rows, const float* __restrict__ scale,
                                                             const float* __restrict__ zero_point,
                                                             const float* __restrict__ obs_min,
                                                             const float* __restrict__ obs_max, int q_type,
                                                             int qmin, int qmax, int16_t* __restrict__ w_int,
                                                             float* __restrict__ w_scale, float* __restrict__ wq,
                                                             uint8_t* __restrict__ pass) {
  int64_t i = (int64_t)blockIdx.x * blockDim.x + threadIdx.x;
  const int64_t stride = (int64_t)gridDim.x * blockDim.x;
  for (; i < n; i += stride) {
    const int r = rows == 1 ? 0 : (int)(i / inner);
    const float s = __ldg(scale + r), zp = __ldg(zero_point + r);
    float a = __fsub_rn(__fdiv_rn(__ldg(obs_min + r), s), zp);
    float b = __fsub_rn(__fdiv_rn(__ldg(obs_max + r), s), zp);
    float lo, hi;
    if (q_type == 0) { hi = fmaxf(fabsf(a), fabsf(b)); lo = -hi; } else { lo = a; hi = b; }
    float v = __fsub_rn(__fdiv_rn(__ldg(w + i), s), zp);
    float rr = mnb_round_half_away(v);
    float c = fminf(fmaxf(rr, (float)qmin), (float)qmax);
    bool ok = !(v > hi) && !(v < lo) && (rr >= (float)qmin) && (rr <= (float)qmax);
    float e = __fadd_rn(c, zp);
    if (wq) wq[i] = __fmul_rn(e, s);
    if (w_int) w_int[i] = (int16_t)fminf(fmaxf(e, -32768.f), 32767.f);
    if (pass) pass[i] = ok ? 1 : 0;
    if (w_scale && i < out_c) w_scale[i] = __ldg(scale + (rows == 1 ? 0 : i));
  }
}

__global__ void __launch_bounds__(256) iao_weight_bwd_kernel(const float* __restrict__ g,
                                                             const uint8_t* __restrict__ pass,
                                                             const float* __restrict__ scale, int64_t n,
                                                             int64_t inner, int rows, float* __restrict__ dw) {
  int64_t i = (int64_t)blockIdx.x * blockDim.x + threadIdx.x;
  const int64_t stride = (int64_t)gridDim.x * blockDim.x;
  for (; i < n; i += stride) {
    const float s = __ldg(scale + (rows == 1 ? 0 : (int)(i / inner)));
    dw[i] = pass[i] ? __fdiv_rn(__fmul_rn(__ldg(g + i), s), s) : 0.f;
  }
}

extern "C" int mnb_iao_weight_fwd(const float* w, int64_t numel, int32_t out_c, int32_t rows, const float* scale,
                                  const float* zero_point, const float* obs_min, const float* obs_max,
                                  int32_t q_type, int32_t qmin, int32_t qmax, int16_t* w_int, float* w_scale,
                                  float* wq, uint8_t* pass, mnb_stream_t stream) {
  MNB_REQUIRE(w && scale && zero_point && obs_min && obs_max && numel > 0, "bad IAO weight arguments");
  MNB_REQUIRE(out_c > 0 && numel % out_c == 0 && (rows == 1 || rows == out_c), "rows must be 1 or out_c");
  int blocks = (int)std::min<int64_t>(mnb_ceil_div(numel, 256), MNB_NUM_SMS * 8);
  iao_weight_fwd_kernel<<<blocks, 256, 0, S(stream)>>>(w, numel, numel / out_c, out_c, rows, scale, zero_point,
                                                        obs_min, obs_max, q_type, qmin, qmax, w_int, w_scale, wq, pass);
  MNB_LAUNCHED(1);
  return 0;
}

extern "C" int mnb_iao_weight_bwd(const float* g_wq, const uint8_t* pass, const float* scale, int64_t numel,
                                  int32_t out_c, int32_t rows, float* dw, mnb_stream_t stream) {
  MNB_REQUIRE(g_wq && pass && scale && dw && numel > 0 && out_c > 0 && numel % out_c == 0, "bad IAO weight-bwd arguments");
  MNB_REQUIRE(rows == 1 || rows == out_c, "rows must be 1 or out_c, got %d for out_c = %d", rows, out_c);
  int blocks = (int)std::min<int64_t>(mnb_ceil_div(numel, 256), MNB_NUM_SMS * 8);
  iao_weight_bwd_kernel<<<blocks, 256, 0, S(stream)>>>(g_wq, pass, scale, numel, numel / out_c, rows, dw);
  MNB_LAUNCHED(1);
  return 0;
}

constexpr int STATS_SPLITS = 32;

struct MnbBnUpdate {
  double eps; float momentum;
  float* running_mean; float* running_var; long long* num_batches_tracked;
};

template <typename XT>
__global__ void __launch_bounds__(256) channel_stats_kernel(const XT* __restrict__ x, const float* __restrict__ dec, int batch,
                                                            int channels, int hw, int as_mean_var, float* __restrict__ stats,
                                                            uint32_t* counters, double* partial, MnbBnUpdate bn) {
  __shared__ double red[32];
  __shared__ bool last;
  const int c = blockIdx.x, sp = blockIdx.y, nsp = gridDim.y;
  const int64_t per = (int64_t)batch * hw;
  double s1 = 0.0, s2 = 0.0;
  const XDec d = x_dec<XT>(dec, channels, c);
  const float pivot = as_mean_var ? x_val<XT>(__ldg(x + (int64_t)c * hw), d) : 0.f;
  const int b_lo = (int)((int64_t)batch * sp / nsp), b_hi = (int)((int64_t)batch * (sp + 1) / nsp);
  const bool vec = (hw & 3) == 0 && ((reinterpret_cast<uintptr_t>(x) & (4 * sizeof(XT) - 1)) == 0);
  if (vec) {
    const uint32_t hw4 = (uint32_t)hw >> 2, total = (uint32_t)(b_hi - b_lo) * hw4;
    float f1[4] = {0.f, 0.f, 0.f, 0.f}, f2[4] = {0.f, 0.f, 0.f, 0.f};
    for (uint32_t t0 = threadIdx.x; t0 < total; t0 += 4 * blockDim.x) {
#pragma unroll
      for (int u = 0; u < 4; ++u) {
        const uint32_t t = t0 + u * blockDim.x;
        if (t < total) {
          const uint32_t b = t / hw4, i = t - b * hw4;
          float4 v = x_load4(x + 4 * (((int64_t)(b_lo + b) * channels + c) * hw4 + i), d);
          v.x -= pivot; v.y -= pivot; v.z -= pivot; v.w -= pivot;
          f1[u] += (v.x + v.y) + (v.z + v.w);
          f2[u] += (v.x * v.x + v.y * v.y) + (v.z * v.z + v.w * v.w);
        }
      }
    }
    s1 = ((double)f1[0] + (double)f1[1]) + ((double)f1[2] + (double)f1[3]);
    s2 = ((double)f2[0] + (double)f2[1]) + ((double)f2[2] + (double)f2[3]);
  } else {
    for (int b = b_lo; b < b_hi; ++b) {
      const XT* plane = x + ((int64_t)b * channels + c) * hw;
      float f1 = 0.f, f2 = 0.f;
      for (int i = threadIdx.x; i < hw; i += blockDim.x) {
        const float v = x_val<XT>(__ldg(plane + i), d) - pivot;
        f1 += v; f2 += v * v;
      }
      s1 += (double)f1;
      s2 += (double)f2;
    }
  }
  s1 = mnb_block_reduce(s1, MnbSum(), 0.0, red);
  s2 = mnb_block_reduce(s2, MnbSum(), 0.0, red);
  if (threadIdx.x == 0) {
    partial[((int64_t)c * nsp + sp) * 2 + 0] = s1;
    partial[((int64_t)c * nsp + sp) * 2 + 1] = s2;
    __threadfence();
    last = (atomicAdd(counters + c, 1u) == (uint32_t)nsp - 1);
  }
  __syncthreads();
  if (!last || threadIdx.x != 0) return;
  __threadfence();
  s1 = 0.0; s2 = 0.0;
  for (int j = 0; j < nsp; ++j) { s1 += partial[((int64_t)c * nsp + j) * 2]; s2 += partial[((int64_t)c * nsp + j) * 2 + 1]; }
  if (as_mean_var) {
    const double dmean = s1 / (double)per;
    double mean = (double)pivot + dmean;
    double ss = s2 - (double)per * dmean * dmean;
    if (ss < 0.0) ss = 0.0;
    double var = ss / (double)(per - 1);
    stats[c] = (float)mean;
    if (as_mean_var == 2) {
      stats[channels + c] = (float)(ss / (double)per);
      stats[2 * channels + c] = (float)var;
    } else if (as_mean_var == 3) {
      stats[channels + c] = (float)(1.0 / sqrt(ss / (double)per + bn.eps));
      const float m = bn.momentum;
      bn.running_mean[c] = __fadd_rn(__fmul_rn(1.f - m, bn.running_mean[c]), __fmul_rn(m, (float)mean));
      bn.running_var[c] = __fadd_rn(__fmul_rn(1.f - m, bn.running_var[c]), __fmul_rn(m, (float)var));
      if (c == 0 && bn.num_batches_tracked) *bn.num_batches_tracked += 1;
    } else {
      stats[channels + c] = (float)var;
    }
  } else {
    stats[c] = (float)s1;
    stats[channels + c] = (float)s2;
  }
  counters[c] = 0;
}

__global__ void __launch_bounds__(256) channel_stats_bwd_kernel(const float* __restrict__ x,
                                                                const float* __restrict__ mean,
                                                                const float* __restrict__ dmean,
                                                                const float* __restrict__ dvar, int batch,
                                                                int channels, int hw, float* __restrict__ dx) {
  const int64_t n = (int64_t)batch * channels * hw;
  const float N = (float)((int64_t)batch * hw);
  int64_t i = (int64_t)blockIdx.x * blockDim.x + threadIdx.x;
  const int64_t stride = (int64_t)gridDim.x * blockDim.x;
  for (; i < n; i += stride) {
    int c = (int)((i / hw) % channels);
    float a = __fdiv_rn(__ldg(dmean + c), N);
    float b = __fmul_rn(__ldg(dvar + c), __fdiv_rn(2.f, N - 1.f));
    dx[i] = __fadd_rn(a, __fmul_rn(b, __fsub_rn(__ldg(x + i), __ldg(mean + c))));
  }
}

extern "C" int mnb_channel_stats(const float* x, int32_t batch, int32_t channels, int32_t hw,
                                 int32_t as_mean_var, float* stats, void* scratch, mnb_stream_t stream) {
  MNB_REQUIRE(x && stats && scratch && batch > 0 && channels > 0 && hw > 0, "bad channel_stats arguments");
  MNB_REQUIRE(channels <= 8192, "channel_stats supports at most 8192 channels, got %d", channels);
  int64_t per = (int64_t)batch * hw;
  int splits = (int)std::max<int64_t>(1, std::min<int64_t>(std::min<int64_t>(STATS_SPLITS, batch), per / 2048));
  splits = std::max(1, std::min(splits, (2 * 8 * MNB_NUM_SMS + channels - 1) / channels));
  uint32_t* counters = reinterpret_cast<uint32_t*>(reinterpret_cast<char*>(scratch) + 16384);
  double* partial = reinterpret_cast<double*>(reinterpret_cast<char*>(scratch) + 49152);
  MNB_REQUIRE(as_mean_var >= 0 && as_mean_var <= 2, "as_mean_var must be 0, 1 or 2");
  channel_stats_kernel<float><<<dim3(channels, splits), 256, 0, S(stream)>>>(x, nullptr, batch, channels, hw, as_mean_var,
                                                                              stats, counters, partial, MnbBnUpdate{});
// ... 246 lines not shown
```

micronet_b200/fused.py:

```python
from __future__ import annotations

import torch
import torch.nn as nn
from torch.autograd import Function

import ctypes as C

import torch.nn.functional as TF

from . import _lib as L
from . import pk as PK


def _xargs(lib, name, x, codes):
    if codes is None:
        return getattr(lib, name), (x.data_ptr(),)
    return getattr(lib, name + "_codes"), (codes[0].data_ptr(), codes[1].data_ptr())


class BNSignFn(Function):

    @staticmethod
    def forward(ctx, x, gamma, beta, mean, invstd, training, shuffle_groups, pool, plane_only=False):
        from . import functional as F_
        lib = L.load()
        x = x.contiguous()
        b, c = x.shape[0], x.shape[1]
        hw = x.numel() // (b * c)
        pk_conv = getattr(x, "_mnb_pk_conv", None)
        codes = getattr(x, "_mnb_codes", None)
        write_plane = L.PK_WBWTAB and c % 8 == 0 and hw % 32 == 0 and x.dim() == 4 and L.PK_MODE != "off"
        if codes is not None and not pool and not write_plane:
            x, codes = F_.materialized(x), None
        bits = torch.empty((x.numel() + 31) // 32, dtype=torch.int32, device=x.device)
        arg = None
        if pool:
            h, w = x.shape[2], x.shape[3]
            y = torch.empty((b, c, h // 2, w // 2), dtype=x.dtype, device=x.device)
            arg = torch.empty(y.numel(), dtype=torch.uint8, device=x.device)
            fn, xa = _xargs(lib, "mnb_bn_sign_pool_fwd", x, codes)
            L.check(fn(*xa, b, c, h, w, mean.data_ptr(), invstd.data_ptr(), gamma.data_ptr(), beta.data_ptr(), shuffle_groups,
                       y.data_ptr(), bits.data_ptr(), arg.data_ptr(), L.stream()), "bn_sign_pool_fwd")
        else:
            y = torch.empty_like(x)
            written = False
            if write_plane:
                plane = torch.empty(x.numel() * 2, dtype=torch.uint8, device=x.device)
                skip_y = bool(plane_only) and L.PLANE_ONLY
                fn, xa = _xargs(lib, "mnb_bn_sign_fwd_packed", x, codes)
                rc = fn(*xa, b, c, hw, mean.data_ptr(), invstd.data_ptr(), gamma.data_ptr(), beta.data_ptr(), shuffle_groups,
                        None if skip_y else y.data_ptr(), bits.data_ptr(), plane.data_ptr(), L.stream())
                if rc == 0:
                    y._mnb_pk_pm1 = plane
                    if skip_y:
                        y._mnb_plane_only = True
                    written = True
                elif rc != L.E_UNSUPPORTED:
                    L.check(rc, "bn_sign_fwd_packed")
                elif codes is not None:
                    x, codes = F_.materialized(x), None
            if not written:
                L.check(lib.mnb_bn_sign_fwd(x.data_ptr(), b, c, hw, mean.data_ptr(), invstd.data_ptr(), gamma.data_ptr(),
                                            beta.data_ptr(), shuffle_groups, y.data_ptr(), bits.data_ptr(), L.stream()),
                        "bn_sign_fwd")
        y._mnb_pm1 = True
        ctx.save_for_backward(x, gamma, mean, invstd)
        ctx.bits, ctx.arg, ctx.training, ctx.shuffle_groups = bits, arg, training, shuffle_groups
        ctx.pk_conv, ctx.codes = pk_conv, codes
        return y

    @staticmethod
    def backward(ctx, g):
        lib = L.load()
        x, gamma, mean, invstd = ctx.saved_tensors
        g = g.contiguous()
        b, c = x.shape[0], x.shape[1]
        hw = x.numel() // (b * c)
        dx = torch.empty_like(x)
        out = torch.empty(3 * c, dtype=torch.float32, device=x.device)
        dgamma, dbeta, dx_sum = out[:c], out[c:2 * c], out[2 * c:]
        scratch = L.scratch(x.device, c)
        if (ctx.arg is not None and ctx.pk_conv is not None and ctx.training and c % 8 == 0 and x.shape[3] % 8 == 0
                and x.shape[2] % 2 == 0):
            w_scale, T = ctx.pk_conv
            fn, xa = _xargs(lib, "mnb_bn_sign_pool_bwd", x, ctx.codes)
            L.check(fn(g.data_ptr(), ctx.bits.data_ptr(), ctx.arg.data_ptr(), *xa, b, c, x.shape[2], x.shape[3],
                       mean.data_ptr(), invstd.data_ptr(), gamma.data_ptr(), 2, ctx.shuffle_groups, dx.data_ptr(),
                       dgamma.data_ptr(), dbeta.data_ptr(), None, scratch.data_ptr(), L.stream()), "bn_sign_pool_bwd (reduce)")
            dy_pk = torch.empty(T * x.numel() * 2, dtype=torch.uint8, device=x.device)
            fn, xa = _xargs(lib, "mnb_bn_sign_pool_bwd_pack", x, ctx.codes)
            L.check(fn(g.data_ptr(), ctx.bits.data_ptr(), ctx.arg.data_ptr(), *xa, b, c, x.shape[2], x.shape[3],
                       mean.data_ptr(), invstd.data_ptr(), gamma.data_ptr(), dgamma.data_ptr(), dbeta.data_ptr(),
                       ctx.shuffle_groups, L.ptr(w_scale), T, dy_pk.data_ptr(), L.stream()), "bn_sign_pool_bwd_pack")
            dx_sum.zero_()
            dx._mnb_pk_dy = (dy_pk, T, w_scale)
        elif ctx.arg is not None:
            fn, xa = _xargs(lib, "mnb_bn_sign_pool_bwd", x, ctx.codes)
            L.check(fn(g.data_ptr(), ctx.bits.data_ptr(), ctx.arg.data_ptr(), *xa, b, c, x.shape[2], x.shape[3],
                       mean.data_ptr(), invstd.data_ptr(), gamma.data_ptr(), 1 if ctx.training else 0, ctx.shuffle_groups,
                       dx.data_ptr(), dgamma.data_ptr(), dbeta.data_ptr(), dx_sum.data_ptr(), scratch.data_ptr(), L.stream()),
                    "bn_sign_pool_bwd")
        elif ctx.pk_conv is not None and ctx.training and c % 8 == 0:
            w_scale, T = ctx.pk_conv
            fn, xa = _xargs(lib, "mnb_bn_sign_bwd", x, ctx.codes)
            L.check(fn(g.data_ptr(), ctx.bits.data_ptr(), *xa, b, c, hw, mean.data_ptr(), invstd.data_ptr(), gamma.data_ptr(),
                       2, ctx.shuffle_groups, dx.data_ptr(), dgamma.data_ptr(), dbeta.data_ptr(), None, scratch.data_ptr(),
                       L.stream()), "bn_sign_bwd (reduce)")
            dy_pk = torch.empty(T * x.numel() * 2, dtype=torch.uint8, device=x.device)
            fn, xa = _xargs(lib, "mnb_bn_sign_bwd_pack", x, ctx.codes)
            L.check(fn(g.data_ptr(), ctx.bits.data_ptr(), *xa, b, c, hw, mean.data_ptr(), invstd.data_ptr(), gamma.data_ptr(),
                       dgamma.data_ptr(), dbeta.data_ptr(), ctx.shuffle_groups, L.ptr(w_scale), T, None, dy_pk.data_ptr(),
                       L.stream()), "bn_sign_bwd_pack")
            dx_sum.zero_()
            dx._mnb_pk_dy = (dy_pk, T, w_scale)
        else:
            fn, xa = _xargs(lib, "mnb_bn_sign_bwd", x, ctx.codes)
            L.check(fn(g.data_ptr(), ctx.bits.data_ptr(), *xa, b, c, hw, mean.data_ptr(), invstd.data_ptr(), gamma.data_ptr(),
                       1 if ctx.training else 0, ctx.shuffle_groups, dx.data_ptr(), dgamma.data_ptr(), dbeta.data_ptr(),
                       dx_sum.data_ptr(), scratch.data_ptr(), L.stream()), "bn_sign_bwd")
        dx._mnb_channel_sum = dx_sum
        return dx, dgamma, dbeta, None, None, None, None, None, None


class BatchNormBinarize2d(nn.BatchNorm2d):

    out_shuffle_groups = 1
    pool2 = False
    plane_only = False

    def forward(self, input):
        L.require_cuda(input, self.weight)
        L.require_f32(input, self.weight)
        assert self.affine and self.track_running_stats and self.momentum is not None, \
            "BatchNormBinarize2d supports affine BN with running statistics and a float momentum"
        if self.training:
            lib = L.load()
            x = input.detach().contiguous()
            b, c = x.shape[0], x.shape[1]
            stats = torch.empty(2 * c, dtype=torch.float32, device=x.device)
            fn, xa = _xargs(lib, "mnb_bn_batch_stats", x, getattr(input, "_mnb_codes", None))
            L.check(fn(*xa, b, c, x.numel() // (b * c), float(self.eps), float(self.momentum), self.running_mean.data_ptr(),
                       self.running_var.data_ptr(), self.num_batches_tracked.data_ptr(), stats.data_ptr(),
                       L.scratch(x.device, c).data_ptr(), L.stream()), "bn_batch_stats")
            mean, invstd = stats[:c], stats[c:]
        else:
            mean = self.running_mean
            invstd = torch.rsqrt(self.running_var + self.eps)
        sg = int(self.out_shuffle_groups)
        if self.pool2 and (input.dim() != 4 or input.shape[2] % 2 or input.shape[3] % 8):
            y = BNSignFn.apply(input, self.weight, self.bias, mean, invstd, self.training, 1, False)
            return MaxPoolFn.apply(y, 2, 2, 0, sg)
        return BNSignFn.apply(input, self.weight, self.bias, mean, invstd, self.training, sg, bool(self.pool2),
                              bool(self.plane_only) and not self.pool2)

    def extra_repr(self):
        return super().extra_repr() + f", pool2={self.pool2}, out_shuffle_groups={self.out_shuffle_groups}"



class BNReluQuantFn(Function):

    @staticmethod
    def forward(ctx, x, gamma, beta, mean, invstd, training, shuffle_groups, a_bits):
        from . import functional as F_
        lib = L.load()
        x = x.contiguous()
        b, c = x.shape[0], x.shape[1]
        hw = x.numel() // (b * c)
        bits = torch.empty((x.numel() + 31) // 32, dtype=torch.int32, device=x.device)
        packed = torch.empty(x.numel() * 2, dtype=torch.uint8, device=x.device)
        qp = F_.ActSpec(L.ACT_DOREFA, bits=a_bits).struct()
        L.check(lib.mnb_bn_relu_quant_pack_fwd(x.data_ptr(), b, c, hw, mean.data_ptr(), invstd.data_ptr(), gamma.data_ptr(),
                                               beta.data_ptr(), C.byref(qp), shuffle_groups, packed.data_ptr(),
                                               bits.data_ptr(), L.stream()), "bn_relu_quant_pack_fwd")
        y = torch.empty_like(x)
        y._mnb_pk_q = (packed, a_bits)
        ctx.save_for_backward(x, gamma, mean, invstd)
        ctx.bits, ctx.training, ctx.shuffle_groups = bits, training, shuffle_groups
        return y

    @staticmethod
    def backward(ctx, g):
        lib = L.load()
        x, gamma, mean, invstd = ctx.saved_tensors
        g = g.contiguous()
        b, c = x.shape[0], x.shape[1]
        hw = x.numel() // (b * c)
        dx = torch.empty_like(x)
        out = torch.empty(3 * c, dtype=torch.float32, device=x.device)
        dgamma, dbeta, dx_sum = out[:c], out[c:2 * c], out[2 * c:]
        L.check(lib.mnb_bn_sign_bwd(g.data_ptr(), ctx.bits.data_ptr(), x.data_ptr(), b, c, hw, mean.data_ptr(),
                                    invstd.data_ptr(), gamma.data_ptr(), 1 if ctx.training else 0, ctx.shuffle_groups,
                                    dx.data_ptr(), dgamma.data_ptr(), dbeta.data_ptr(), dx_sum.data_ptr(),
                                    L.scratch(x.device, c).data_ptr(), L.stream()), "bn_sign_bwd")
        dx._mnb_channel_sum = dx_sum
# ... 327 lines not shown
```

Baseline: 41620.

## Add one-launch L2-chunked BN backward reduce+pack and deepen stats loads

Adds a one-launch BatchNorm-sign backward that processes the plane in L2-sized chunks. It computes the dgamma/dbeta reduction and then packs the dy pieces while the data is still resident in L2, avoiding a second DRAM read of g and x. This path is gated behind an environment variable that defaults off, and falls back to the two-kernel path when unsupported. The reduce and channel-stats kernels also batch several vector loads before consuming them, to raise memory-level parallelism at the cost of more registers.

```diff
diff --git a/harness/bn_chunk_probe.py b/harness/bn_chunk_probe.py
--- /dev/null
+++ b/harness/bn_chunk_probe.py
@@ -0,0 +1,97 @@
+import argparse
+import json
+import subprocess
+import statistics
+
+import torch
+
+from micronet_b200 import _lib as L
+
+MB = 1 << 20
+PLANES = [("L1", 256, 1024, 2), ("L3", 512, 256, 16), ("L4", 512, 256, 4), ("L6", 1024, 64, 32), ("L7", 1024, 64, 1)]
+BUDGETS = [8, 12, 16, 24, 32]
+B, T, SETS, PER_WINDOW, WINDOWS = 256, 2, 4, 50, 5
+
+
+def card():
+    try:
+        return subprocess.run(["nvidia-smi", "--query-gpu=name,power.limit,clocks.max.sm", "--format=csv,noheader"],
+                              capture_output=True, text=True, timeout=30).stdout.strip()
+    except (OSError, subprocess.SubprocessError):
+        return torch.cuda.get_device_name(0)
+
+
+def operands(Cc, hw, seed):
+    g = torch.Generator(device="cuda").manual_seed(seed)
+    n = B * Cc * hw
+    return dict(g=torch.randn(n, generator=g, device="cuda"),
+                x=torch.randint(-3000, 3000, (n,), generator=g, device="cuda", dtype=torch.int32).to(torch.int16),
+                dec=torch.cat([torch.rand(Cc, generator=g, device="cuda") * 1e-3, torch.randn(Cc, generator=g, device="cuda")]),
+                bits=torch.randint(0, 2 ** 31 - 1, ((n + 31) // 32,), generator=g, device="cuda", dtype=torch.int32),
+                mean=torch.zeros(Cc, device="cuda"), invstd=torch.ones(Cc, device="cuda"),
+                gamma=torch.rand(Cc, generator=g, device="cuda") + 0.5, scale=torch.rand(Cc, generator=g, device="cuda") + 0.5,
+                dx=torch.empty(n, device="cuda"), dgb=torch.empty(2 * Cc, device="cuda"),
+                pieces=torch.empty(T * n * 2, dtype=torch.uint8, device="cuda"))
+
+
+def two_pass(lib, o, Cc, hw, sg, scratch):
+    L.check(lib.mnb_bn_sign_bwd_codes(o["g"].data_ptr(), o["bits"].data_ptr(), o["x"].data_ptr(), o["dec"].data_ptr(), B, Cc,
+                                      hw, o["mean"].data_ptr(), o["invstd"].data_ptr(), o["gamma"].data_ptr(), 2, sg,
+                                      o["dx"].data_ptr(), o["dgb"].data_ptr(), o["dgb"][Cc:].data_ptr(), None, scratch,
+                                      L.stream()), "bn_sign_bwd_codes")
+    L.check(lib.mnb_bn_sign_bwd_pack_codes(o["g"].data_ptr(), o["bits"].data_ptr(), o["x"].data_ptr(), o["dec"].data_ptr(), B,
+                                           Cc, hw, o["mean"].data_ptr(), o["invstd"].data_ptr(), o["gamma"].data_ptr(),
+                                           o["dgb"].data_ptr(), o["dgb"][Cc:].data_ptr(), sg, o["scale"].data_ptr(), T, None,
+                                           o["pieces"].data_ptr(), L.stream()), "bn_sign_bwd_pack_codes")
+
+
+def one_launch(lib, o, Cc, hw, sg, scratch, budget):
+    L.check(lib.mnb_bn_sign_bwd_pack_l2_codes(o["g"].data_ptr(), o["bits"].data_ptr(), o["x"].data_ptr(), o["dec"].data_ptr(),
+                                              B, Cc, hw, o["mean"].data_ptr(), o["invstd"].data_ptr(), o["gamma"].data_ptr(), sg,
+                                              o["scale"].data_ptr(), T, None, o["dgb"].data_ptr(), o["dgb"][Cc:].data_ptr(),
+                                              o["pieces"].data_ptr(), scratch, budget, L.stream()), "bn_sign_bwd_pack_l2_codes")
+
+
+def window(fn, sets):
+    a, b = torch.cuda.Event(enable_timing=True), torch.cuda.Event(enable_timing=True)
+    a.record()
+    for i in range(PER_WINDOW):
+        fn(sets[i % SETS])
+    b.record()
+    b.synchronize()
+    return a.elapsed_time(b) * 1000.0 / PER_WINDOW
+
+
+def main():
+    ap = argparse.ArgumentParser()
+    ap.add_argument("--out", default=None)
+    args = ap.parse_args()
+    lib = L.load()
+    rows = []
+    print(card())
+    for name, Cc, hw, sg in PLANES:
+        sets = [operands(Cc, hw, 100 + s) for s in range(SETS)]
+        scratch = L.scratch(torch.device("cuda"), Cc).data_ptr()
+        n = B * Cc * hw
+        bytes_two_pass = 2 * (n * 4 + n * 2 + n / 8) + T * n * 2
+        fns = {"two-pass": lambda o: two_pass(lib, o, Cc, hw, sg, scratch)}
+        for mb in BUDGETS:
+            fns[f"{mb} MB"] = lambda o, mb=mb: one_launch(lib, o, Cc, hw, sg, scratch, mb * MB)
+        for fn in fns.values():
+            fn(sets[0])
+        torch.cuda.synchronize()
+        times = {k: [] for k in fns}
+        for _ in range(WINDOWS):
+            for k, fn in fns.items():
+                times[k].append(window(fn, sets))
+        for k, ts in times.items():
+            us = statistics.median(ts)
+            rows.append(dict(plane=name, C=Cc, hw=hw, sg=sg, variant=k, us=round(us, 1), gbs=round(bytes_two_pass / us / 1e3, 0)))
+            print(f"{name} C={Cc} hw={hw} sg={sg} {k:>9}: {us:8.1f} us  {bytes_two_pass / us / 1e3:6.0f} GB/s")
+    if args.out:
+        with open(args.out, "w") as f:
+            json.dump(dict(card=card(), rows=rows), f, indent=1)
+
+
+if __name__ == "__main__":
+    main()
diff --git a/harness/step_profile.py b/harness/step_profile.py
--- a/harness/step_profile.py
+++ b/harness/step_profile.py
@@ -1,4 +1,5 @@
 import argparse
+import ctypes
 import json
 import os
 import re
@@ -38,6 +39,8 @@
         out["bn_sign_bwd_reduce_kernel"] = n * xb + 4 * n + bits
         if pk_conv:
             out["bn_sign_bwd_pack_kernel"] = n * xb + 4 * n + bits + 2 * n * terms_dy
+            if rec.get("l2"):
+                out["bn_bwd_l2_pack_kernel"] = out.pop("bn_sign_bwd_reduce_kernel") + out.pop("bn_sign_bwd_pack_kernel")
         else:
             out["bn_sign_bwd_apply_kernel"] = n * xb + 4 * n + bits + 4 * n
     return out
@@ -72,11 +75,20 @@
 
     calls = []
 
+    def one_launch_bwd(x):
+        if L.BN_L2CHUNK_MB <= 0 or x.dim() != 4:
+            return False
+        out = (ctypes.c_int32 * 8)()
+        b, c = x.shape[0], x.shape[1]
+        xb = 2 if getattr(x, "_mnb_codes", None) is not None else 4
+        L.check(L.load().mnb_bn_bwd_l2_plan(b, c, x.numel() // (b * c), xb, L.BN_L2CHUNK_MB << 20, out, 8), "bn_bwd_l2_plan")
+        return out[0] > 0
+
     def hook(mod, inp):
         x = inp[0]
         calls.append({"n": x.numel(), "xb": 2 if getattr(x, "_mnb_codes", None) is not None else 4,
                       "pool2": bool(mod.pool2), "plane_only": bool(mod.plane_only) and not mod.pool2,
-                      "pk_conv": getattr(x, "_mnb_pk_conv", None) is not None})
+                      "pk_conv": getattr(x, "_mnb_pk_conv", None) is not None, "l2": one_launch_bwd(x)})
 
     handles = [m.register_forward_pre_hook(hook) for m in model.modules() if isinstance(m, BatchNormBinarize2d)]
     acts = [torch.profiler.ProfilerActivity.CPU, torch.profiler.ProfilerActivity.CUDA]
diff --git a/include/micronet_b200.h b/include/micronet_b200.h
--- a/include/micronet_b200.h
+++ b/include/micronet_b200.h
@@ -209,6 +209,17 @@
                                     const float* invstd, const float* gamma, const float* dgamma, const float* dbeta,
                                     int32_t out_shuffle_groups, const float* ch_scale, int32_t terms, void* dy_packed,
                                     mnb_stream_t stream);
+int mnb_bn_sign_bwd_pack_l2(const float* g, const uint32_t* pass_bits, const float* x, int32_t batch, int32_t channels, int32_t hw,
+                            const float* mean, const float* invstd, const float* gamma, int32_t out_shuffle_groups,
+                            const float* ch_scale, int32_t terms, float* dx, float* dgamma, float* dbeta, void* dy_packed,
+                            void* scratch, int64_t budget_bytes, mnb_stream_t stream);
+int mnb_bn_sign_bwd_pack_l2_codes(const float* g, const uint32_t* pass_bits, const int16_t* codes, const float* dec,
+                                  int32_t batch, int32_t channels, int32_t hw, const float* mean, const float* invstd,
+                                  const float* gamma, int32_t out_shuffle_groups, const float* ch_scale, int32_t terms, float* dx,
+                                  float* dgamma, float* dbeta, void* dy_packed, void* scratch, int64_t budget_bytes,
+                                  mnb_stream_t stream);
+int mnb_bn_bwd_l2_plan(int32_t batch, int32_t channels, int32_t hw, int32_t x_bytes, int64_t budget_bytes, int32_t* out,
+                       int32_t n);
 int mnb_pk_pack_act_relu(const float* x, int32_t batch, int32_t channels, int32_t h, int32_t w, const mnb_act_qparams* qp,
                          int32_t terms, const float* ch_scale, int32_t phase_split, int32_t relu, void* out_pk,
                          uint8_t* bits8, mnb_stream_t stream);
diff --git a/micronet_b200/_lib.py b/micronet_b200/_lib.py
--- a/micronet_b200/_lib.py
+++ b/micronet_b200/_lib.py
@@ -120,6 +120,10 @@
     "mnb_bn_sign_pool_fwd_codes": (C.c_int, [_P, _P, _I, _I, _I, _I, _P, _P, _P, _P, _I, _P, _P, _P, _P]),
     "mnb_bn_sign_pool_bwd_codes": (C.c_int, [_P, _P, _P, _P, _P, _I, _I, _I, _I, _P, _P, _P, _I, _I, _P, _P, _P, _P, _P, _P]),
     "mnb_bn_sign_bwd_pack_codes": (C.c_int, [_P, _P, _P, _P, _I, _I, _I, _P, _P, _P, _P, _P, _I, _P, _I, _P, _P, _P]),
+    "mnb_bn_sign_bwd_pack_l2": (C.c_int, [_P, _P, _P, _I, _I, _I, _P, _P, _P, _I, _P, _I, _P, _P, _P, _P, _P, _L, _P]),
+    "mnb_bn_sign_bwd_pack_l2_codes": (C.c_int, [_P, _P, _P, _P, _I, _I, _I, _P, _P, _P, _I, _P, _I, _P, _P, _P, _P, _P, _L,
+                                                _P]),
+    "mnb_bn_bwd_l2_plan": (C.c_int, [_I, _I, _I, _I, _L, _P, _I]),
     "mnb_bn_sign_pool_bwd_pack_codes": (C.c_int, [_P, _P, _P, _P, _P, _I, _I, _I, _I, _P, _P, _P, _P, _P, _I, _P, _I, _P,
                                                   _P]),
     "mnb_quant_add_pack_fwd": (C.c_int, [_P, _P, _I, _I, _I, _I, _ACTQ, _I, _P, C.POINTER(PkPost), _P]),
@@ -247,6 +251,7 @@
 PK_WBWTAB = os.environ.get("MNB_PK_WBWTAB", "1") == "1"
 PK_WG_TAPS = os.environ.get("MNB_PK_WG_TAPS", "1") != "0"
 PK_GC3 = os.environ.get("MNB_PK_GC3", "1") != "0"
+BN_L2CHUNK_MB = int(os.environ.get("MNB_BN_L2CHUNK", "0"))
 
 XNOR_MODE = os.environ.get("MNB_XNOR", "auto")
 
diff --git a/micronet_b200/csrc/mnb_bn_bwd.cuh b/micronet_b200/csrc/mnb_bn_bwd.cuh
--- /dev/null
+++ b/micronet_b200/csrc/mnb_bn_bwd.cuh
@@ -0,0 +1,104 @@
+#pragma once
+#include <algorithm>
+
+#include "mnb_common.cuh"
+
+constexpr int FUSED_SPLITS = 32;
+
+__device__ __forceinline__ uint32_t shuffled_channel(uint32_t c, uint32_t sg, uint32_t cpg) {
+  return sg > 1 ? (c % cpg) * sg + c / cpg : c;
+}
+
+static inline int plane_splits(int batch, int64_t per, int channels) {
+  const int64_t want = (2 * 8 * MNB_NUM_SMS + channels - 1) / channels;
+  return (int)std::max<int64_t>(1, std::min<int64_t>(std::min<int64_t>(std::min<int64_t>(FUSED_SPLITS, batch), per / 2048), want));
+}
+
+template <bool VEC, int DEPTH, typename XT>
+__device__ __forceinline__ bool bn_sign_bwd_reduce_item(int c, int sp, int nsp, const float* __restrict__ g,
+                                                        const uint32_t* __restrict__ bits, const XT* __restrict__ x,
+                                                        const float* __restrict__ dec, int batch, int channels, int hw, int sg,
+                                                        const float* __restrict__ mean, const float* __restrict__ invstd,
+                                                        float* __restrict__ dgamma, float* __restrict__ dbeta,
+                                                        uint32_t* counters, double* partial) {
+  __shared__ double red[32];
+  __shared__ bool last;
+  const int oc = (int)shuffled_channel((uint32_t)c, (uint32_t)sg, (uint32_t)(channels / sg));
+  const float mu = __ldg(mean + c), is = __ldg(invstd + c);
+  const XDec d = x_dec<XT>(dec, channels, c);
+  const int b_lo = (int)((int64_t)batch * sp / nsp), b_hi = (int)((int64_t)batch * (sp + 1) / nsp);
+  double s1, s2;
+  if (VEC) {
+    const uint32_t hw4 = (uint32_t)hw >> 2, total = (uint32_t)(b_hi - b_lo) * hw4;
+    const float4* g4 = reinterpret_cast<const float4*>(g);
+    float f1[2] = {0.f, 0.f}, f2[2] = {0.f, 0.f};
+    for (uint32_t t0 = threadIdx.x; t0 < total; t0 += 2 * DEPTH * blockDim.x) {
+      float4 gv[DEPTH][2], xv[DEPTH][2];
+      uint32_t nib[DEPTH][2];
+#pragma unroll
+      for (int q = 0; q < DEPTH; ++q)
+#pragma unroll
+        for (int u = 0; u < 2; ++u) {
+          const uint32_t t = t0 + (2 * q + u) * blockDim.x;
+          if (t < total) {
+            const uint32_t b = t / hw4, i = t - b * hw4;
+            const uint32_t fi4 = ((uint32_t)(b_lo + b) * channels + c) * hw4 + i;
+            const uint32_t go4 = ((uint32_t)(b_lo + b) * channels + oc) * hw4 + i;
+            nib[q][u] = (__ldg(bits + (fi4 >> 3)) >> (4 * (fi4 & 7))) & 15u;
+            gv[q][u] = __ldg(g4 + go4);
+            xv[q][u] = x_load4(x + 4 * fi4, d);
+          }
+        }
+#pragma unroll
+      for (int q = 0; q < DEPTH; ++q)
+#pragma unroll
+        for (int u = 0; u < 2; ++u) {
+          const uint32_t t = t0 + (2 * q + u) * blockDim.x;
+          if (t < total) {
+            const uint32_t nb = nib[q][u];
+            const float4 gq = gv[q][u], xq = xv[q][u];
+            const float g0 = (nb & 1u) ? gq.x : 0.f, g1 = (nb & 2u) ? gq.y : 0.f, g2 = (nb & 4u) ? gq.z : 0.f,
+                        g3 = (nb & 8u) ? gq.w : 0.f;
+            f1[u] += (g0 + g1) + (g2 + g3);
+            f2[u] += (g0 * ((xq.x - mu) * is) + g1 * ((xq.y - mu) * is)) + (g2 * ((xq.z - mu) * is) + g3 * ((xq.w - mu) * is));
+          }
+        }
+    }
+    s1 = (double)f1[0] + (double)f1[1];
+    s2 = (double)f2[0] + (double)f2[1];
+  } else {
+    s1 = 0.0; s2 = 0.0;
+    for (int b = b_lo; b < b_hi; ++b) {
+      const int64_t off = ((int64_t)b * channels + c) * hw, goff = ((int64_t)b * channels + oc) * hw;
+      float f1 = 0.f, f2 = 0.f;
+      for (int i = threadIdx.x; i < hw; i += blockDim.x) {
+        const int64_t fi = off + i;
+        const bool pass = (__ldg(bits + (fi >> 5)) >> (fi & 31)) & 1u;
+        const float gv = pass ? __ldg(g + goff + i) : 0.f;
+        f1 += gv;
+        f2 += gv * ((x_val<XT>(__ldg(x + fi), d) - mu) * is);
+      }
+      s1 += (double)f1; s2 += (double)f2;
+    }
+  }
+  s1 = mnb_block_reduce(s1, MnbSum(), 0.0, red);
+  s2 = mnb_block_reduce(s2, MnbSum(), 0.0, red);
+  if (threadIdx.x == 0) {
+    partial[((int64_t)c * nsp + sp) * 2 + 0] = s1;
+    partial[((int64_t)c * nsp + sp) * 2 + 1] = s2;
+    __threadfence();
+    last = (atomicAdd(counters + c, 1u) == (uint32_t)nsp - 1);
+  }
+  __syncthreads();
+  if (!last || threadIdx.x != 0) return false;
+  __threadfence();
+  s1 = 0.0; s2 = 0.0;
+  for (int j = 0; j < nsp; ++j) {
+    s1 += __ldcg(partial + ((int64_t)c * nsp + j) * 2);
+    s2 += __ldcg(partial + ((int64_t)c * nsp + j) * 2 + 1);
+  }
+  dbeta[c] = (float)s1;
+  dgamma[c] = (float)s2;
+  counters[c] = 0;
+  return true;
+}
diff --git a/micronet_b200/csrc/mnb_common.cuh b/micronet_b200/csrc/mnb_common.cuh
--- a/micronet_b200/csrc/mnb_common.cuh
+++ b/micronet_b200/csrc/mnb_common.cuh
@@ -23,6 +23,7 @@
 
 static inline int mnb_ceil_div(int64_t a, int64_t b) { return (int)((a + b - 1) / b); }
 constexpr int MNB_NUM_SMS = 132;
+constexpr int MNB_SCRATCH_CHUNK_SYNC = 14336;
 
 
 __device__ __forceinline__ float mnb_round_half_away(float v) {
diff --git a/micronet_b200/csrc/mnb_fused.cu b/micronet_b200/csrc/mnb_fused.cu
--- a/micronet_b200/csrc/mnb_fused.cu
+++ b/micronet_b200/csrc/mnb_fused.cu
@@ -1,13 +1,9 @@
 #include <algorithm>
 
+#include "mnb_bn_bwd.cuh"
 #include "mnb_common.cuh"
 
 static inline cudaStream_t S(mnb_stream_t s) { return (cudaStream_t)s; }
-constexpr int FUSED_SPLITS = 32;
-
-__device__ __forceinline__ uint32_t shuffled_channel(uint32_t c, uint32_t sg, uint32_t cpg) {
-  return sg > 1 ? (c % cpg) * sg + c / cpg : c;
-}
 
 __global__ void __launch_bounds__(256) bn_sign_fwd_v4_kernel(const float4* __restrict__ x, uint32_t n4, uint32_t channels,
                                                              uint32_t hw4, uint32_t sg, const float* __restrict__ mean,
@@ -74,68 +70,8 @@
                                                                  const float* __restrict__ invstd, float* __restrict__ dgamma,
                                                                  float* __restrict__ dbeta, uint32_t* counters,
                                                                  double* partial) {
-  __shared__ double red[32];
-  __shared__ bool last;
-  const int c = blockIdx.x, sp = blockIdx.y, nsp = gridDim.y;
-  const int oc = (int)shuffled_channel((uint32_t)c, (uint32_t)sg, (uint32_t)(channels / sg));
-  const float mu = __ldg(mean + c), is = __ldg(invstd + c);
-  const XDec d = x_dec<XT>(dec, channels, c);
-  const int b_lo = (int)((int64_t)batch * sp / nsp), b_hi = (int)((int64_t)batch * (sp + 1) / nsp);
-  double s1, s2;
-  if (VEC) {
-    const uint32_t hw4 = (uint32_t)hw >> 2, total = (uint32_t)(b_hi - b_lo) * hw4;
-    const float4* g4 = reinterpret_cast<const float4*>(g);
-    float f1[2] = {0.f, 0.f}, f2[2] = {0.f, 0.f};
-    for (uint32_t t0 = threadIdx.x; t0 < total; t0 += 2 * blockDim.x) {
-#pragma unroll
-      for (int u = 0; u < 2; ++u) {
-        const uint32_t t = t0 + u * blockDim.x;
-        if (t < total) {
-          const uint32_t b = t / hw4, i = t - b * hw4;
-          const uint32_t fi4 = ((uint32_t)(b_lo + b) * channels + c) * hw4 + i;
-          const uint32_t go4 = ((uint32_t)(b_lo + b) * channels + oc) * hw4 + i;
-          const uint32_t nib = (__ldg(bits + (fi4 >> 3)) >> (4 * (fi4 & 7))) & 15u;
-          const float4 gv = __ldg(g4 + go4), xv = x_load4(x + 4 * fi4, d);
-          const float g0 = (nib & 1u) ? gv.x : 0.f, g1 = (nib & 2u) ? gv.y : 0.f, g2 = (nib & 4u) ? gv.z : 0.f,
-                      g3 = (nib & 8u) ? gv.w : 0.f;
-          f1[u] += (g0 + g1) + (g2 + g3);
-          f2[u] += (g0 * ((xv.x - mu) * is) + g1 * ((xv.y - mu) * is)) + (g2 * ((xv.z - mu) * is) + g3 * ((xv.w - mu) * is));
-        }
-      }
-    }
-    s1 = (double)f1[0] + (double)f1[1];
-    s2 = (double)f2[0] + (double)f2[1];
-  } else {
-    s1 = 0.0; s2 = 0.0;
-    for (int b = b_lo; b < b_hi; ++b) {
-      const int64_t off = ((int64_t)b * channels + c) * hw, goff = ((int64_t)b * channels + oc) * hw;
-      float f1 = 0.f, f2 = 0.f;
-      for (int i = threadIdx.x; i < hw; i += blockDim.x) {
-        const int64_t fi = off + i;
-        const bool pass = (__ldg(bits + (fi >> 5)) >> (fi & 31)) & 1u;
-        const float gv = pass ? __ldg(g + goff + i) : 0.f;
-        f1 += gv;
-        f2 += gv * ((x_val<XT>(__ldg(x + fi), d) - mu) * is);
-      }
-      s1 += (double)f1; s2 += (double)f2;
-    }
-  }
-  s1 = mnb_block_reduce(s1, MnbSum(), 0.0, red);
-  s2 = mnb_block_reduce(s2, MnbSum(), 0.0, red);
-  if (threadIdx.x == 0) {
-    partial[((int64_t)c * nsp + sp) * 2 + 0] = s1;
-    partial[((int64_t)c * nsp + sp) * 2 + 1] = s2;
-    __threadfence();
-    last = (atomicAdd(counters + c, 1u) == (uint32_t)nsp - 1);
-  }
-  __syncthreads();
-  if (!last || threadIdx.x != 0) return;
-  __threadfence();
-  s1 = 0.0; s2 = 0.0;
-  for (int j = 0; j < nsp; ++j) { s1 += partial[((int64_t)c * nsp + j) * 2]; s2 += partial[((int64_t)c * nsp + j) * 2 + 1]; }
-  dbeta[c] = (float)s1;
-  dgamma[c] = (float)s2;
-  counters[c] = 0;
+  bn_sign_bwd_reduce_item<VEC, 1, XT>(blockIdx.x, blockIdx.y, gridDim.y, g, bits, x, dec, batch, channels, hw, sg, mean, invstd,
+                                      dgamma, dbeta, counters, partial);
 }
 
 template <bool VEC, typename XT>
@@ -225,11 +161,6 @@
   return (hw & 3) == 0 && n < (1ll << 31) &&
          (((uintptr_t)a | (uintptr_t)b | (uintptr_t)c) & 15) == 0 && ((uintptr_t)x & (4 * sizeof(XT) - 1)) == 0;
 }
-static int plane_splits(int batch, int64_t per, int channels) {
-  const int64_t want = (2 * 8 * MNB_NUM_SMS + channels - 1) / channels;
-  return (int)std::max<int64_t>(1, std::min<int64_t>(std::min<int64_t>(std::min<int64_t>(FUSED_SPLITS, batch), per / 2048), want));
-}
-
 extern "C" int mnb_bn_sign_fwd(const float* x, int32_t batch, int32_t channels, int32_t hw, const float* mean,
                                const float* invstd, const float* gamma, const float* beta, int32_t out_shuffle_groups,
                                float* y, uint32_t* pass_bits, mnb_stream_t stream) {
diff --git a/micronet_b200/csrc/mnb_pk.cu b/micronet_b200/csrc/mnb_pk.cu
--- a/micronet_b200/csrc/mnb_pk.cu
+++ b/micronet_b200/csrc/mnb_pk.cu
@@ -5,6 +5,7 @@
 #include <cstdlib>
 #include <cstring>
 
+#include "mnb_bn_bwd.cuh"
 #include "mnb_common.cuh"
 #include "mnb_tc.cuh"
 
@@ -673,21 +674,27 @@
 template <> struct PkVec<2> { typedef float2 type; };
 template <> struct PkVec<4> { typedef float4 type; };
 
-template <int VEC, typename XT>
-__global__ void __launch_bounds__(256) bn_sign_bwd_pack_kernel(const float* __restrict__ g, const uint32_t* __restrict__ bits,
-                                                               const XT* __restrict__ x, const float* __restrict__ dec,
-                                                               int batch, int channels, int hw,
-                                                               int sg, float inv_count, const float* __restrict__ mean,
-                                                               const float* __restrict__ invstd, const float* __restrict__ gamma,
-                                                               const float* __restrict__ dgamma, const float* __restrict__ dbeta,
-                                                               const float* __restrict__ ch_scale, int terms,
-                                                               float* __restrict__ dx, uint4* __restrict__ out, int64_t plane_vecs) {
+template <typename XT>
+struct BwdPackArgs {
+  const float* g; const uint32_t* bits; const XT* x; const float* dec;
+  int batch, channels, hw, sg; float inv_count;
+  const float *mean, *invstd, *gamma, *dgamma, *dbeta, *ch_scale;
+  int terms; float* dx; uint4* out; int64_t plane_vecs;
+};
+
+template <int VEC, typename XT, bool L2_STATS = false>
+__device__ __forceinline__ void bn_sign_bwd_pack_warp(int64_t w, const BwdPackArgs<XT>& a) {
   typedef typename PkVec<VEC>::type T;
   const int lane = threadIdx.x & 31;
+  const float* __restrict__ g = a.g; const uint32_t* __restrict__ bits = a.bits; const XT* __restrict__ x = a.x;
+  const float* __restrict__ dec = a.dec; const float* __restrict__ mean = a.mean; const float* __restrict__ invstd = a.invstd;
+  const float* __restrict__ gamma = a.gamma; const float* __restrict__ ch_scale = a.ch_scale;
+  const int channels = a.channels, hw = a.hw, sg = a.sg, terms = a.terms;
+  const float inv_count = a.inv_count;
+  float* __restrict__ dx = a.dx;
+  uint4* __restrict__ out = a.out;
   const int c8n = channels / 8, cpg = channels / sg, chunks = hw / (32 * VEC);
-  const int64_t items = (int64_t)batch * c8n * chunks;
-  const int64_t nwarps = ((int64_t)gridDim.x * blockDim.x) >> 5;
-  for (int64_t w = ((int64_t)blockIdx.x * blockDim.x + threadIdx.x) >> 5; w < items; w += nwarps) {
+  {
     const int ch = (int)(w % chunks);
     const int64_t pl = w / chunks;
     const int c8 = (int)(pl % c8n), b = (int)(pl / c8n);
@@ -709,7 +716,8 @@
     for (int j = 0; j < 8; ++j) {
       const int c = c8 * 8 + j;
       const float mu = __ldg(mean + c), is = __ldg(invstd + c), k = __ldg(gamma + c) * is;
-      const float db = __ldg(dbeta + c) * inv_count, dg = __ldg(dgamma + c) * inv_count;
+      const float db = (L2_STATS ? __ldcg(a.dbeta + c) : __ldg(a.dbeta + c)) * inv_count;
+      const float dg = (L2_STATS ? __ldcg(a.dgamma + c) : __ldg(a.dgamma + c)) * inv_count;
       const float sc = ch_scale ? __ldg(ch_scale + c) : 1.f;
       const float* gf = reinterpret_cast<const float*>(&gv[j]);
       T dv;
@@ -735,8 +743,97 @@
           v[i][2 * j] -= __uint_as_float(pk4[j] << 16);
           v[i][2 * j + 1] -= __uint_as_float(pk4[j] & 0xffff0000u);
         }
-        out[(int64_t)tm * plane_vecs + dst + i] = make_uint4(pk4[0], pk4[1], pk4[2], pk4[3]);
+        out[(int64_t)tm * a.plane_vecs + dst + i] = make_uint4(pk4[0], pk4[1], pk4[2], pk4[3]);
       }
+    }
+  }
+}
+
+template <int VEC, typename XT>
+__global__ void __launch_bounds__(256) bn_sign_bwd_pack_kernel(const BwdPackArgs<XT> a) {
+  const int64_t items = (int64_t)a.batch * (a.channels / 8) * (a.hw / (32 * VEC));
+  const int64_t nwarps = ((int64_t)gridDim.x * blockDim.x) >> 5;
+  for (int64_t w = ((int64_t)blockIdx.x * blockDim.x + threadIdx.x) >> 5; w < items; w += nwarps) bn_sign_bwd_pack_warp<VEC, XT>(w, a);
+}
+
+constexpr int L2_AW = 4;
+constexpr int L2_MAX_CHUNKS = 510;
+
+struct L2Chunks {
+  int K, q8, splits, hwc;
+  uint32_t nR, nA, nRl, nAl;
+};
+
+__device__ __forceinline__ uint32_t ld_acquire_gpu(const uint32_t* p) {
+  uint32_t v;
+  asm volatile("ld.acquire.gpu.global.u32 %0, [%1];" : "=r"(v) : "l"(p) : "memory");
+  return v;
+}
+
+template <int VEC, typename XT>
+__global__ void __launch_bounds__(256) bn_bwd_l2_pack_kernel(const BwdPackArgs<XT> a, const L2Chunks p, uint32_t* sync,
+                                                             uint32_t* counters, double* partial) {
+  __shared__ uint32_t s_ticket;
+  uint32_t* done = sync + 2;
+  const int c8n = a.channels / 8;
+  const uint32_t pair = p.nR + p.nA, mid = (uint32_t)(p.K - 2) * pair;
+  const uint32_t total = p.nR + mid + p.nRl + p.nA + p.nAl;
+  for (;;) {
+    if (threadIdx.x == 0) s_ticket = atomicAdd(sync, 1u);
+    __syncthreads();
+    uint32_t t = s_ticket;
+    __syncthreads();
+    if (t >= total) break;
+    int k;
+    bool apply;
+    if (t < p.nR) {
+      k = 0; apply = false;
+    } else if ((t -= p.nR) < mid) {
+      k = 1 + (int)(t / pair); t %= pair;
+      apply = t >= p.nR;
+      if (apply) { t -= p.nR; k -= 1; }
+    } else if ((t -= mid) < p.nRl) {
+      k = p.K - 1; apply = false;
+    } else if ((t -= p.nRl) < p.nA) {
+      k = p.K - 2; apply = true;
+    } else {
+      t -= p.nA; k = p.K - 1; apply = true;
+    }
+    const int c8lo = k * p.q8, nq = min(c8n - c8lo, p.q8);
+    if (!apply) {
+      const int c = c8lo * 8 + (int)(t / (uint32_t)p.splits), sp = (int)(t % (uint32_t)p.splits);
+      if (bn_sign_bwd_reduce_item<true, 4, XT>(c, sp, p.splits, a.g, a.bits, a.x, a.dec, a.batch, a.channels, a.hw, a.sg, a.mean,
+                                               a.invstd, const_cast<float*>(a.dgamma), const_cast<float*>(a.dbeta), counters,
+                                               partial)) {
+        __threadfence();
+        atomicAdd(done + k, 1u);
+      }
+    } else {
+      if (threadIdx.x == 0) {
+        const uint32_t need = 8u * (uint32_t)nq;
+        while (ld_acquire_gpu(done + k) < need) __nanosleep(128);
+      }
+      __syncthreads();
+      const int64_t wk = (int64_t)a.batch * nq * p.hwc;
+#pragma unroll 1
+      for (int j = 0; j < L2_AW; ++j) {
+        const int64_t i = ((int64_t)t * L2_AW + j) * 8 + (threadIdx.x >> 5);
+        if (i < wk) {
+          const int ch = (int)(i % p.hwc);
+          const int64_t r = i / p.hwc;
+          const int c8 = c8lo + (int)(r % nq), b = (int)(r / nq);
+          bn_sign_bwd_pack_warp<VEC, XT, true>(((int64_t)b * c8n + c8) * p.hwc + ch, a);
+        }
+      }
+    }
+  }
+  if (threadIdx.x == 0) {
+    __threadfence();
+    if (atomicAdd(sync + 1, 1u) == gridDim.x - 1) {
+      for (int k = 0; k < p.K; ++k) done[k] = 0;
+      sync[0] = 0;
+      sync[1] = 0;
+      __threadfence();
     }
   }
 }
@@ -2177,6 +2274,24 @@
 }
 
 template <typename XT>
+static int bwd_pack_vec(int hw, const float* g, const XT* x, const float* dx) {
+  auto al = [](const void* p, int a) { return p == nullptr || (reinterpret_cast<uintptr_t>(p) & (uintptr_t)(a - 1)) == 0; };
+  constexpr int xs = (int)sizeof(XT);
+  return (hw % 128 == 0 && al(g, 16) && al(x, 4 * xs) && al(dx, 16)) ? 4
+         : ((hw % 64 == 0 && al(g, 8) && al(x, 2 * xs) && al(dx, 8)) ? 2 : 1);
+}
+
+template <typename XT>
+static pk::BwdPackArgs<XT> bwd_pack_args(const float* g, const uint32_t* pass_bits, const XT* x, const float* dec, int batch,
+                                         int channels, int hw, const float* mean, const float* invstd, const float* gamma,
+                                         const float* dgamma, const float* dbeta, int sg, const float* ch_scale, int terms,
+                                         float* dx, void* dy_packed) {
+  return pk::BwdPackArgs<XT>{g, pass_bits, x, dec, batch, channels, hw, sg, 1.f / (float)((int64_t)batch * hw), mean, invstd,
+                             gamma, dgamma, dbeta, ch_scale, terms, dx, reinterpret_cast<uint4*>(dy_packed),
+                             (int64_t)batch * (channels / 8) * hw};
+}
+
+template <typename XT>
 static int bn_sign_bwd_pack(const float* g, const uint32_t* pass_bits, const XT* x, const float* dec, int32_t batch,
                             int32_t channels, int32_t hw, const float* mean, const float* invstd, const float* gamma,
                             const float* dgamma, const float* dbeta, int32_t out_shuffle_groups, const float* ch_scale,
@@ -2189,22 +2304,15 @@
     return mnb_fail(MNB_E_UNSUPPORTED, "packed BatchNorm backward needs channels %% 8 == 0 and a 16-byte aligned output");
   if (hw % 32) return mnb_fail(MNB_E_UNSUPPORTED, "packed BatchNorm backward needs H*W %% 32 == 0");
   const int c8n = channels / 8;
-  auto al = [](const void* p, int a) { return p == nullptr || (reinterpret_cast<uintptr_t>(p) & (uintptr_t)(a - 1)) == 0; };
-  constexpr int xs = (int)sizeof(XT);
-  const int vec = (hw % 128 == 0 && al(g, 16) && al(x, 4 * xs) && al(dx, 16)) ? 4
-                  : ((hw % 64 == 0 && al(g, 8) && al(x, 2 * xs) && al(dx, 8)) ? 2 : 1);
+  const int vec = bwd_pack_vec(hw, g, x, dx);
   const int64_t warps = (int64_t)batch * c8n * (hw / (32 * vec));
   const int blocks = (int)std::min<int64_t>(mnb_ceil_div(warps, 8), (int64_t)MNB_NUM_SMS * 8);
-  const float inv_count = 1.f / (float)((int64_t)batch * hw);
-  uint4* outp = reinterpret_cast<uint4*>(dy_packed);
-  const int64_t plane_vecs = (int64_t)batch * c8n * hw;
+  const pk::BwdPackArgs<XT> a = bwd_pack_args(g, pass_bits, x, dec, batch, channels, hw, mean, invstd, gamma, dgamma, dbeta,
+                                               out_shuffle_groups, ch_scale, terms, dx, dy_packed);
   cudaStream_t st = (cudaStream_t)stream;
-#define MNB_BWD_PACK(V)                                                                                                          \
-  pk::bn_sign_bwd_pack_kernel<V, XT><<<blocks, 256, 0, st>>>(g, pass_bits, x, dec, batch, channels, hw, out_shuffle_groups,     \
-                                                             inv_count, mean, invstd, gamma, dgamma, dbeta, ch_scale, terms, dx, \
-                                                             outp, plane_vecs)
-  if (vec == 4) MNB_BWD_PACK(4); else if (vec == 2) MNB_BWD_PACK(2); else MNB_BWD_PACK(1);
-#undef MNB_BWD_PACK
+  if (vec == 4) pk::bn_sign_bwd_pack_kernel<4, XT><<<blocks, 256, 0, st>>>(a);
+  else if (vec == 2) pk::bn_sign_bwd_pack_kernel<2, XT><<<blocks, 256, 0, st>>>(a);
+  else pk::bn_sign_bwd_pack_kernel<1, XT><<<blocks, 256, 0, st>>>(a);
   MNB_LAUNCHED(1);
   return 0;
 }
@@ -2224,6 +2332,102 @@
   MNB_REQUIRE(dec, "NULL decode pair");
   return bn_sign_bwd_pack<int16_t>(g, pass_bits, codes, dec, batch, channels, hw, mean, invstd, gamma, dgamma, dbeta,
                                    out_shuffle_groups, ch_scale, terms, dx, dy_packed, stream);
+}
+
+static bool bwd_l2_plan(int batch, int channels, int hw, int x_bytes, int vec, int64_t budget, pk::L2Chunks& p) {
+  const int c8n = channels / 8;
+  const int64_t octet_bytes = (int64_t)8 * batch * hw * (4 + x_bytes) + (int64_t)batch * hw;
+  p.q8 = (int)std::max<int64_t>(1, std::min<int64_t>(c8n, budget / octet_bytes));
+  p.K = (c8n + p.q8 - 1) / p.q8;
+  if (budget <= 0 || p.K < 2 || p.K > pk::L2_MAX_CHUNKS) return false;
+  p.splits = plane_splits(batch, (int64_t)batch * hw, channels);
+  p.hwc = hw / (32 * vec);
+  const int ql = c8n - (p.K - 1) * p.q8;
+  const int64_t wpi = (int64_t)8 * pk::L2_AW;
+  p.nR = (uint32_t)(8 * p.q8 * p.splits);
+  p.nRl = (uint32_t)(8 * ql * p.splits);
+  p.nA = (uint32_t)mnb_ceil_div((int64_t)batch * p.q8 * p.hwc, wpi);
+  p.nAl = (uint32_t)mnb_ceil_div((int64_t)batch * ql * p.hwc, wpi);
+  return true;
+}
+
+extern "C" int mnb_bn_bwd_l2_plan(int32_t batch, int32_t channels, int32_t hw, int32_t x_bytes, int64_t budget, int32_t* out,
+                                  int32_t n) {
+  MNB_REQUIRE(out && n >= 8 && batch > 0 && channels > 0 && hw > 0 && (x_bytes == 2 || x_bytes == 4), "bad bn_bwd_l2_plan arguments");
+  for (int i = 0; i < 8; ++i) out[i] = 0;
+  if (channels % 8 || hw % 32) return 0;
+  const int vec = hw % 128 == 0 ? 4 : (hw % 64 == 0 ? 2 : 1);
+  pk::L2Chunks p;
+  if (!bwd_l2_plan(batch, channels, hw, x_bytes, vec, budget, p)) return 0;
+  const int32_t v[8] = {p.K, p.q8, p.splits, vec, (int32_t)p.nR, (int32_t)p.nA, (int32_t)p.nRl, (int32_t)p.nAl};
+  for (int i = 0; i < 8; ++i) out[i] = v[i];
+  return 0;
+}
+
+template <int VEC, typename XT>
+static int launch_bwd_l2(const pk::BwdPackArgs<XT>& a, const pk::L2Chunks& p, uint32_t* sync, uint32_t* counters, double* partial,
+                         cudaStream_t st) {
+  static int per_sm = 0;
+  if (per_sm == 0) {
+    cudaError_t e = cudaOccupancyMaxActiveBlocksPerMultiprocessor(&per_sm, pk::bn_bwd_l2_pack_kernel<VEC, XT>, 256, 0);
+    if (e != cudaSuccess || per_sm < 1) return mnb_fail((int)e, "occupancy of bn_bwd_l2_pack_kernel: %s", cudaGetErrorString(e));
+  }
+  const int grid = (int)std::min<int64_t>((int64_t)per_sm * MNB_NUM_SMS, (int64_t)p.nR + p.nA);
+  pk::bn_bwd_l2_pack_kernel<VEC, XT><<<grid, 256, 0, st>>>(a, p, sync, counters, partial);
+  MNB_LAUNCHED(1);
+  return 0;
+}
+
+template <typename XT>
+static int bn_sign_bwd_pack_l2(const float* g, const uint32_t* pass_bits, const XT* x, const float* dec, int32_t batch,
+                               int32_t channels, int32_t hw, const float* mean, const float* invstd, const float* gamma,
+                               int32_t out_shuffle_groups, const float* ch_scale, int32_t terms, float* dx, float* dgamma,
+                               float* dbeta, void* dy_packed, void* scratch, int64_t budget, mnb_stream_t stream) {
+  MNB_REQUIRE(g && pass_bits && x && mean && invstd && gamma && dgamma && dbeta && dy_packed && scratch,
+              "NULL bn_sign_bwd_pack_l2 pointer");
+  MNB_REQUIRE(batch > 0 && channels > 0 && channels <= 8192 && hw > 0 && terms >= 1 && terms <= 3,
+              "bad bn_sign_bwd_pack_l2 arguments");
+  MNB_REQUIRE(out_shuffle_groups >= 1 && channels % out_shuffle_groups == 0, "shuffle groups %d do not divide %d channels",
+              out_shuffle_groups, channels);
+  const bool vec_reduce = (hw & 3) == 0 && (int64_t)batch * channels * hw < (1ll << 31) &&
+                          ((reinterpret_cast<uintptr_t>(g) | reinterpret_cast<uintptr_t>(dx)) & 15) == 0 &&
+                          (reinterpret_cast<uintptr_t>(x) & (4 * sizeof(XT) - 1)) == 0;
+  if (channels % 8 || hw % 32 || (reinterpret_cast<uintptr_t>(dy_packed) & 15) || !vec_reduce)
+    return mnb_fail(MNB_E_UNSUPPORTED, "one-launch BatchNorm backward needs channels %% 8 == 0, H*W %% 32 == 0, < 2^31 "
+                                       "elements, aligned tensors");
+  const int vec = bwd_pack_vec(hw, g, x, dx);
+  pk::L2Chunks p;
+  if (!bwd_l2_plan(batch, channels, hw, (int)sizeof(XT), vec, budget, p))
+    return mnb_fail(MNB_E_UNSUPPORTED, "one-launch BatchNorm backward: the plane is one chunk of a %lld-byte budget",
+                    (long long)budget);
+  const pk::BwdPackArgs<XT> a = bwd_pack_args(g, pass_bits, x, dec, batch, channels, hw, mean, invstd, gamma, dgamma, dbeta,
+                                               out_shuffle_groups, ch_scale, terms, dx, dy_packed);
+  char* sb = reinterpret_cast<char*>(scratch);
+  uint32_t* sync = reinterpret_cast<uint32_t*>(sb + MNB_SCRATCH_CHUNK_SYNC);
+  uint32_t* counters = reinterpret_cast<uint32_t*>(sb + 16384);
+  double* partial = reinterpret_cast<double*>(sb + 49152);
+  cudaStream_t st = (cudaStream_t)stream;
+  if (vec == 4) return launch_bwd_l2<4, XT>(a, p, sync, counters, partial, st);
+  if (vec == 2) return launch_bwd_l2<2, XT>(a, p, sync, counters, partial, st);
+  return launch_bwd_l2<1, XT>(a, p, sync, counters, partial, st);
+}
+
+extern "C" int mnb_bn_sign_bwd_pack_l2(const float* g, const uint32_t* pass_bits, const float* x, int32_t batch, int32_t channels,
+                                       int32_t hw, const float* mean, const float* invstd, const float* gamma,
+                                       int32_t out_shuffle_groups, const float* ch_scale, int32_t terms, float* dx, float* dgamma,
+                                       float* dbeta, void* dy_packed, void* scratch, int64_t budget_bytes, mnb_stream_t stream) {
+  return bn_sign_bwd_pack_l2<float>(g, pass_bits, x, nullptr, batch, channels, hw, mean, invstd, gamma, out_shuffle_groups,
+                                    ch_scale, terms, dx, dgamma, dbeta, dy_packed, scratch, budget_bytes, stream);
+}
+
+extern "C" int mnb_bn_sign_bwd_pack_l2_codes(const float* g, const uint32_t* pass_bits, const int16_t* codes, const float* dec,
+                                             int32_t batch, int32_t channels, int32_t hw, const float* mean, const float* invstd,
+                                             const float* gamma, int32_t out_shuffle_groups, const float* ch_scale, int32_t terms,
+                                             float* dx, float* dgamma, float* dbeta, void* dy_packed, void* scratch,
+                                             int64_t budget_bytes, mnb_stream_t stream) {
+  MNB_REQUIRE(dec, "NULL decode pair");
+  return bn_sign_bwd_pack_l2<int16_t>(g, pass_bits, codes, dec, batch, channels, hw, mean, invstd, gamma, out_shuffle_groups,
+                                      ch_scale, terms, dx, dgamma, dbeta, dy_packed, scratch, budget_bytes, stream);
 }
 
 template <typename XT>
diff --git a/micronet_b200/csrc/mnb_quant.cu b/micronet_b200/csrc/mnb_quant.cu
--- a/micronet_b200/csrc/mnb_quant.cu
+++ b/micronet_b200/csrc/mnb_quant.cu
@@ -592,6 +592,7 @@
 }
 
 constexpr int STATS_SPLITS = 32;
+constexpr int STATS_DEPTH = 2;
 
 struct MnbBnUpdate {
   double eps; float momentum;
@@ -612,20 +613,35 @@
   const int b_lo = (int)((int64_t)batch * sp / nsp), b_hi = (int)((int64_t)batch * (sp + 1) / nsp);
   const bool vec = (hw & 3) == 0 && ((reinterpret_cast<uintptr_t>(x) & (4 * sizeof(XT) - 1)) == 0);
   if (vec) {
+    typedef typename XVec<XT>::t4 R4;
+    const R4* xr = reinterpret_cast<const R4*>(x);
     const uint32_t hw4 = (uint32_t)hw >> 2, total = (uint32_t)(b_hi - b_lo) * hw4;
     float f1[4] = {0.f, 0.f, 0.f, 0.f}, f2[4] = {0.f, 0.f, 0.f, 0.f};
-    for (uint32_t t0 = threadIdx.x; t0 < total; t0 += 4 * blockDim.x) {
+    for (uint32_t t0 = threadIdx.x; t0 < total; t0 += 4 * STATS_DEPTH * blockDim.x) {
+      R4 raw[STATS_DEPTH][4];
 #pragma unroll
-      for (int u = 0; u < 4; ++u) {
-        const uint32_t t = t0 + u * blockDim.x;
-        if (t < total) {
-          const uint32_t b = t / hw4, i = t - b * hw4;
-          float4 v = x_load4(x + 4 * (((int64_t)(b_lo + b) * channels + c) * hw4 + i), d);
-          v.x -= pivot; v.y -= pivot; v.z -= pivot; v.w -= pivot;
-          f1[u] += (v.x + v.y) + (v.z + v.w);
-          f2[u] += (v.x * v.x + v.y * v.y) + (v.z * v.z + v.w * v.w);
+      for (int q = 0; q < STATS_DEPTH; ++q)
+#pragma unroll
+        for (int u = 0; u < 4; ++u) {
+          const uint32_t t = t0 + (4 * q + u) * blockDim.x;
+          if (t < total) {
+            const uint32_t b = t / hw4, i = t - b * hw4;
+            raw[q][u] = __ldg(xr + (((int64_t)(b_lo + b) * channels + c) * hw4 + i));
+          }
         }
-      }
+#pragma unroll
+      for (int q = 0; q < STATS_DEPTH; ++q)
+#pragma unroll
+        for (int u = 0; u < 4; ++u) {
+          const uint32_t t = t0 + (4 * q + u) * blockDim.x;
+          if (t < total) {
+            const R4 r = raw[q][u];
+            float4 v = make_float4(x_val<XT>(r.x, d), x_val<XT>(r.y, d), x_val<XT>(r.z, d), x_val<XT>(r.w, d));
+            v.x -= pivot; v.y -= pivot; v.z -= pivot; v.w -= pivot;
+            f1[u] += (v.x + v.y) + (v.z + v.w);
+            f2[u] += (v.x * v.x + v.y * v.y) + (v.z * v.z + v.w * v.w);
+          }
+        }
     }
     s1 = ((double)f1[0] + (double)f1[1]) + ((double)f1[2] + (double)f1[3]);
     s2 = ((double)f2[0] + (double)f2[1]) + ((double)f2[2] + (double)f2[3]);
diff --git a/micronet_b200/fused.py b/micronet_b200/fused.py
--- a/micronet_b200/fused.py
+++ b/micronet_b200/fused.py
@@ -102,15 +102,24 @@
                     "bn_sign_pool_bwd")
         elif ctx.pk_conv is not None and ctx.training and c % 8 == 0:
             w_scale, T = ctx.pk_conv
-            fn, xa = _xargs(lib, "mnb_bn_sign_bwd", x, ctx.codes)
-            L.check(fn(g.data_ptr(), ctx.bits.data_ptr(), *xa, b, c, hw, mean.data_ptr(), invstd.data_ptr(), gamma.data_ptr(),
-                       2, ctx.shuffle_groups, dx.data_ptr(), dgamma.data_ptr(), dbeta.data_ptr(), None, scratch.data_ptr(),
-                       L.stream()), "bn_sign_bwd (reduce)")
             dy_pk = torch.empty(T * x.numel() * 2, dtype=torch.uint8, device=x.device)
-            fn, xa = _xargs(lib, "mnb_bn_sign_bwd_pack", x, ctx.codes)
-            L.check(fn(g.data_ptr(), ctx.bits.data_ptr(), *xa, b, c, hw, mean.data_ptr(), invstd.data_ptr(), gamma.data_ptr(),
-                       dgamma.data_ptr(), dbeta.data_ptr(), ctx.shuffle_groups, L.ptr(w_scale), T, None, dy_pk.data_ptr(),
-                       L.stream()), "bn_sign_bwd_pack")
+            rc = L.E_UNSUPPORTED
+            if L.BN_L2CHUNK_MB > 0:
+                fn, xa = _xargs(lib, "mnb_bn_sign_bwd_pack_l2", x, ctx.codes)
+                rc = fn(g.data_ptr(), ctx.bits.data_ptr(), *xa, b, c, hw, mean.data_ptr(), invstd.data_ptr(), gamma.data_ptr(),
+                        ctx.shuffle_groups, L.ptr(w_scale), T, None, dgamma.data_ptr(), dbeta.data_ptr(), dy_pk.data_ptr(),
+                        scratch.data_ptr(), L.BN_L2CHUNK_MB << 20, L.stream())
+                if rc != L.E_UNSUPPORTED:
+                    L.check(rc, "bn_sign_bwd_pack_l2")
+            if rc != 0:
+                fn, xa = _xargs(lib, "mnb_bn_sign_bwd", x, ctx.codes)
+                L.check(fn(g.data_ptr(), ctx.bits.data_ptr(), *xa, b, c, hw, mean.data_ptr(), invstd.data_ptr(),
+                           gamma.data_ptr(), 2, ctx.shuffle_groups, dx.data_ptr(), dgamma.data_ptr(), dbeta.data_ptr(), None,
+                           scratch.data_ptr(), L.stream()), "bn_sign_bwd (reduce)")
+                fn, xa = _xargs(lib, "mnb_bn_sign_bwd_pack", x, ctx.codes)
+                L.check(fn(g.data_ptr(), ctx.bits.data_ptr(), *xa, b, c, hw, mean.data_ptr(), invstd.data_ptr(),
+                           gamma.data_ptr(), dgamma.data_ptr(), dbeta.data_ptr(), ctx.shuffle_groups, L.ptr(w_scale), T, None,
+                           dy_pk.data_ptr(), L.stream()), "bn_sign_bwd_pack")
             dx_sum.zero_()
             dx._mnb_pk_dy = (dy_pk, T, w_scale)
         else:
```

Result: faster. 42250 (median of 6 runs) (+1.5%).
